# tum-pbs/PhiFlow

Measured on NVIDIA H100. Metric: smoke_plume_512^3_steps_per_sec, higher is better.
Workload: dtype f32

## Files before the change

phiflow_b200/csrc/ring_kernels.cu:

```cuda
#include <cooperative_groups.h>
#include <type_traits>
#include "cg_common.cuh"
#include <cstdlib>
#include <cstring>
#include "launch.cuh"

namespace cg = cooperative_groups;

#define RING_CONSUMERS 256
#define RING_THREADS (RING_CONSUMERS + 32)
#define RING_MAX_STAGES 8
#define RING_G 4

struct RingCfg {
    int TY, R, pitch, nx4;
    int stage_floats;
    int ZC, nyt, nzc;
    int units_per_batch, total_units;
    int consumers;
    int groups;
    int shfl_ok;
    int hint;
    int merge;
    int dbg;
    int split, Zm, split_t;
};

__device__ __forceinline__ uint32_t smem_u32(const void* p) { return (uint32_t)__cvta_generic_to_shared(p); }
__device__ __forceinline__ void mbar_init(uint32_t bar, uint32_t count)
{ asm volatile("mbarrier.init.shared::cta.b64 [%0], %1;" ::"r"(bar), "r"(count) : "memory"); }
__device__ __forceinline__ void mbar_expect_tx(uint32_t bar, uint32_t bytes)
{ asm volatile("mbarrier.arrive.expect_tx.shared::cta.b64 _, [%0], %1;" ::"r"(bar), "r"(bytes) : "memory"); }
__device__ __forceinline__ void mbar_arrive(uint32_t bar)
{ asm volatile("mbarrier.arrive.shared::cta.b64 _, [%0];" ::"r"(bar) : "memory"); }
__device__ __forceinline__ void mbar_wait(uint32_t bar, uint32_t parity)
{
    asm volatile(
        "{\n"
        ".reg .pred p;\n"
        "WAIT_LOOP:\n"
        "mbarrier.try_wait.parity.shared::cta.b64 p, [%0], %1;\n"
        "@p bra.uni WAIT_DONE;\n"
        "bra.uni WAIT_LOOP;\n"
        "WAIT_DONE:\n"
        "}\n" ::"r"(bar), "r"(parity) : "memory");
}
__device__ __forceinline__ void bulk_g2s(uint32_t dst, const void* src, uint32_t bytes, uint32_t bar)
{
    asm volatile("cp.async.bulk.shared::cluster.global.mbarrier::complete_tx::bytes [%0], [%1], %2, [%3];"
                 ::"r"(dst), "l"(src), "r"(bytes), "r"(bar) : "memory");
}
__device__ __forceinline__ void bulk_g2s_stream(uint32_t dst, const void* src, uint32_t bytes, uint32_t bar)
{
    uint64_t pol;
    asm volatile("createpolicy.fractional.L2::evict_first.b64 %0, 1.0;" : "=l"(pol));
    asm volatile("cp.async.bulk.shared::cluster.global.mbarrier::complete_tx::bytes.L2::cache_hint [%0], [%1], %2, [%3], %4;"
                 ::"r"(dst), "l"(src), "r"(bytes), "r"(bar), "l"(pol) : "memory");
}
__device__ __forceinline__ void fence_proxy_async() { asm volatile("fence.proxy.async;" ::: "memory"); }

struct SlotIt {
    int slot; unsigned par;
    __device__ __forceinline__ void next(int R) { if (++slot == R) { slot = 0; par ^= 1u; } }
};

struct Ring {
    float* stage0;
    uint32_t stage0_s, full0, empty0;
    SlotIt pos;
};

__device__ __forceinline__ void ring_init(Ring& rg, unsigned char* smem, const RingCfg& cfg)
{
    uint64_t* bars = reinterpret_cast<uint64_t*>(smem);
    rg.full0 = smem_u32(bars);
    rg.empty0 = smem_u32(bars + RING_MAX_STAGES);
    rg.stage0 = reinterpret_cast<float*>(smem + 128);
    rg.stage0_s = smem_u32(rg.stage0);
    rg.pos.slot = 0; rg.pos.par = 0;
    if (threadIdx.x == 0) {
        for (int s = 0; s < cfg.R; ++s) {
            mbar_init(rg.full0 + 8 * s, 1);
            mbar_init(rg.empty0 + 8 * s, cfg.consumers / 32);
        }
        asm volatile("fence.mbarrier_init.release.cluster;" ::: "memory");
    }
    __syncthreads();
}

struct ProdUnit {
    long long yoff[4];
    const float* base[4];
    uint32_t dsto[4];
    uint32_t nbytes[4];
    unsigned hmask, emask;
    int tot_h, tot_e;
};

template <int DIM, bool KSLOT = false>
__device__ __forceinline__ void prod_unit_setup(ProdUnit& pu, const RingCfg& cfg, const DGrid& g, const DField& pf,
                                                unsigned hactive, int NHslots, int NE, const float* const* hsrc, const float* const* esrc,
                                                int b, int y0, int kb = 0)
{
    const int lane = threadIdx.x & 31, hrows = cfg.TY + 2;
    const uint32_t row_bytes = (uint32_t)cfg.pitch * 4u;
    const bool mergeable = cfg.merge && pf.sy == cfg.pitch;
    pu.hmask = pu.emask = 0;
    int ch = 0, ce = 0;
#pragma unroll
    for (int it = 0; it < 4; ++it) {
        const int r = lane + 32 * it;
        pu.yoff[it] = 0; pu.base[it] = nullptr; pu.dsto[it] = 0; pu.nbytes[it] = row_bytes;
        int key = -1, yv = 0;
        bool halo_line = false;
        if (r < NHslots * hrows) {
            const int arr = r / hrows, j = r - arr * hrows;
            int yy = y0 - 1 + j; float cv;
            if (((hactive >> arr) & 1u) && yy <= g.n[1] && phi_resolve(yy, pf, 1, cv)) {
                pu.yoff[it] = (long long)((KSLOT && arr == NHslots - 1) ? kb : b) * pf.sb + (long long)yy * pf.sy;
                pu.base[it] = hsrc[arr];
                pu.dsto[it] = 4u * (uint32_t)((arr * hrows + j) * cfg.pitch);
                key = arr; yv = yy; halo_line = true; ch++;
            }
        } else if (r < NHslots * hrows + NE * cfg.TY) {
            const int q = r - NHslots * hrows, arr = q / cfg.TY, j = q - arr * cfg.TY;
            const int yy = y0 + j;
            if (yy < g.n[1]) {
                pu.yoff[it] = (long long)b * pf.sb + (long long)yy * pf.sy;
                pu.base[it] = esrc[arr];
                pu.dsto[it] = 4u * (uint32_t)((NHslots * hrows + arr * cfg.TY + j) * cfg.pitch);
                key = 8 + arr; yv = yy; ce++;
            }
        }
        const int pkey = __shfl_up_sync(0xffffffffu, key, 1), pyv = __shfl_up_sync(0xffffffffu, yv, 1);
        const bool cont = mergeable && key >= 0 && lane > 0 && pkey == key && pyv + 1 == yv;
        const unsigned cm = __ballot_sync(0xffffffffu, cont);
        if (key >= 0 && !cont) {
            const unsigned follow = lane == 31 ? 0u : (cm >> (lane + 1));
            pu.nbytes[it] = (uint32_t)__ffs(~follow) * row_bytes;
            if (halo_line) pu.hmask |= 1u << it; else pu.emask |= 1u << it;
        }
    }
#pragma unroll
    for (int o = 16; o > 0; o >>= 1) { ch += __shfl_xor_sync(0xffffffffu, ch, o); ce += __shfl_xor_sync(0xffffffffu, ce, o); }
    pu.tot_h = ch; pu.tot_e = ce;
}

template <int DIM>
__device__ __forceinline__ void ring_produce(Ring& rg, const RingCfg& cfg, const DField& pf, const ProdUnit& pu, int z, bool interior)
{
    const int lane = threadIdx.x & 31;
    const int slot = rg.pos.slot;
    const uint32_t full = rg.full0 + 8 * slot;
    const uint32_t row_bytes = (uint32_t)cfg.pitch * 4u;
    const uint32_t sbase = rg.stage0_s + 4u * (uint32_t)(slot * cfg.stage_floats);
    float cv;
    bool zmem = true;
    if (DIM == 3) zmem = phi_resolve(z, pf, 2, cv); else z = 0;
    const long long zoff = (long long)z * pf.sz;
    unsigned mask = (zmem ? pu.hmask : 0u) | (interior ? pu.emask : 0u);
    const int cnt = (zmem ? pu.tot_h : 0) + (interior ? pu.tot_e : 0);
    if (lane == 0) {
        mbar_wait(rg.empty0 + 8 * slot, rg.pos.par ^ 1u);
        if (cnt > 0) mbar_expect_tx(full, (uint32_t)cnt * row_bytes); else mbar_arrive(full);
    }
    __syncwarp();
#pragma unroll
    for (int it = 0; it < 4; ++it)
        if (mask & (1u << it)) {
            if (cfg.hint && (pu.emask & (1u << it))) bulk_g2s_stream(sbase + pu.dsto[it], pu.base[it] + pu.yoff[it] + zoff, pu.nbytes[it], full);
            else bulk_g2s(sbase + pu.dsto[it], pu.base[it] + pu.yoff[it] + zoff, pu.nbytes[it], full);
        }
    rg.pos.next(cfg.R);
}

__device__ __forceinline__ void ring_wait_full(const Ring& rg, const SlotIt& s) { mbar_wait(rg.full0 + 8 * s.slot, s.par); }
__device__ __forceinline__ void ring_release(const Ring& rg, const SlotIt& s)
{
    __syncwarp();
    if ((threadIdx.x & 31) == 0) mbar_arrive(rg.empty0 + 8 * s.slot);
}
__device__ __forceinline__ const float* ring_ptr(const Ring& rg, const RingCfg& cfg, const SlotIt& s)
{ return rg.stage0 + (size_t)s.slot * cfg.stage_floats; }

#define GF_VALID 1u
#define GF_XLO   2u
#define GF_XHI   4u
#define GF_YLOC  8u
#define GF_YHIC  16u

struct ThreadGroups {
    int soff[RING_G];
    int eoff[RING_G];
    int goff[RING_G];
    int j[RING_G];
    int xlo[RING_G], xro[RING_G];
    unsigned needl, needr;
    unsigned flags[RING_G];
    bool fast_ok;
};

__device__ __forceinline__ void groups_init(ThreadGroups& tg, const RingCfg& cfg, const DGrid& g, const DField& pf)
{
    const int lane = threadIdx.x & 31, nx = g.n[0];
    tg.needl = tg.needr = 0;
#pragma unroll
    for (int k = 0; k < RING_G; ++k) {
        const int gi = threadIdx.x + k * cfg.consumers;
        const int j = gi / cfg.nx4, x0 = (gi - j * cfg.nx4) * 4;
        tg.j[k] = (k < cfg.groups && j < cfg.TY && x0 < nx) ? j : -1;
        tg.soff[k] = (j + 1) * cfg.pitch + x0;
        tg.eoff[k] = j * cfg.pitch + x0;
        tg.goff[k] = j * (int)pf.sy + x0;
        tg.flags[k] = 0;
        const int row = (j + 1) * cfg.pitch;
        tg.xlo[k] = tg.soff[k] - 1; tg.xro[k] = tg.soff[k] + 4;
        if (lane == 0) tg.needl |= 1u << k;
        if (lane == 31) tg.needr |= 1u << k;
        if (x0 == 0) { tg.needl |= 1u << k; tg.xlo[k] = pf.klo[0] == PHI_BC_PERIODIC ? row + nx - 1 : row; }
        if (x0 + 4 >= nx) { tg.needr |= 1u << k; tg.xro[k] = pf.khi[0] == PHI_BC_PERIODIC ? row : row + nx - 1; }
        if (!(tg.needl & (1u << k))) tg.xlo[k] = 0;
        if (!(tg.needr & (1u << k))) tg.xro[k] = 0;
    }
    tg.fast_ok = cfg.shfl_ok && (cfg.nx4 * 4 == nx) && (cfg.TY * cfg.nx4 == cfg.groups * cfg.consumers)
                 && pf.klo[0] != PHI_BC_CONST && pf.khi[0] != PHI_BC_CONST;
}

__device__ __forceinline__ void groups_tile(ThreadGroups& tg, const RingCfg& cfg, const DGrid& g, const DField& pf, int y0)
{
    const int nx = g.n[0], ny = g.n[1];
#pragma unroll
    for (int k = 0; k < RING_G; ++k) {
        unsigned f = 0;
        if (tg.j[k] >= 0) {
            const int y = y0 + tg.j[k];
            const int x0 = tg.eoff[k] - tg.j[k] * cfg.pitch;
            if (y < ny) {
                f = GF_VALID;
                if (x0 == 0) f |= GF_XLO;
                if (x0 + 4 >= nx) f |= GF_XHI;
                if (y == 0 && pf.klo[1] == PHI_BC_CONST) f |= GF_YLOC;
                if (y == ny - 1 && pf.khi[1] == PHI_BC_CONST) f |= GF_YHIC;
            }
        }
        tg.flags[k] = f;
    }
}

template <int DIM, int NH, int NE, CgOp OP = CgOp::Poisson, class Epi>
__device__ __forceinline__ void ring_compute(const RingCfg& cfg, const DGrid& g, const DField& pf, const ThreadGroups& tg,
                                             const float* sm, const float* sc, const float* sp, float beta,
                                             long long plane_off, int z, Epi& epi, const CgOperator* od)
{
    const int pitch = cfg.pitch;
    const int h1 = (cfg.TY + 2) * pitch;
    const int aoff = NH * (cfg.TY + 2) * pitch;
    const int e0off = (NH + (cg_op_xslot(OP) ? 1 : 0)) * (cfg.TY + 2) * pitch;
    const int e1off = e0off + cfg.TY * pitch;
    const float ix2 = g.inv_dx2[0], iy2 = g.inv_dx2[1], iz2 = g.inv_dx2[2];
    const bool zm_const = DIM == 3 && z == 0 && pf.klo[2] == PHI_BC_CONST;
    const bool zp_const = DIM == 3 && z == g.n[2] - 1 && pf.khi[2] == PHI_BC_CONST;
    const bool use1 = NH == 2 && beta != 0.f;
    const int lane = threadIdx.x & 31;

    auto val4 = [&](const float* s, int off) -> float4 {
        float4 a = *reinterpret_cast<const float4*>(s + off);
        if (use1) { const float4 o = *reinterpret_cast<const float4*>(s + h1 + off);
                    a.x = fmaf(beta, o.x, a.x); a.y = fmaf(beta, o.y, a.y); a.z = fmaf(beta, o.z, a.z); a.w = fmaf(beta, o.w, a.w); }
        return a;
    };
    auto val1 = [&](const float* s, int off) -> float {
        float a = s[off];
        if (use1) a = fmaf(beta, s[h1 + off], a);
        return a;
    };

#pragma unroll
    for (int k = 0; k < RING_G; ++k) {
        const unsigned f = tg.flags[k];
        const int rc = tg.soff[k];
        const bool valid = (f & GF_VALID) != 0;
        float4 c = f4_splat(0.f);
        if (valid) c = val4(sc, rc);
        float xl, xr;
        if (cfg.shfl_ok) {
            xl = __shfl_up_sync(0xffffffffu, c.w, 1);
            xr = __shfl_down_sync(0xffffffffu, c.x, 1);
            if (valid && lane == 0 && !(f & GF_XLO)) xl = val1(sc, rc - 1);
            if (valid && lane == 31 && !(f & GF_XHI)) xr = val1(sc, rc + 4);
        } else if (valid) {
            xl = (f & GF_XLO) ? 0.f : val1(sc, rc - 1);
            xr = (f & GF_XHI) ? 0.f : val1(sc, rc + 4);
        }
        if (!valid) continue;
        float4 ym, yp, q;
        int nvalid = 4;
        if (f == GF_VALID) {
            ym = val4(sc, rc - pitch);
            yp = val4(sc, rc + pitch);
        } else {
            const int row = rc - (tg.eoff[k] - tg.j[k] * pitch);
            const int nx = g.n[0];
            const int x0 = rc - row;
            nvalid = min(4, nx - x0);
            ym = (f & GF_YLOC) ? f4_splat(pf.clo[1]) : val4(sc, rc - pitch);
            yp = (f & GF_YHIC) ? f4_splat(pf.chi[1]) : val4(sc, rc + pitch);
            if (f & GF_XLO) { const int kx = pf.klo[0]; xl = kx == PHI_BC_PERIODIC ? val1(sc, row + nx - 1) : (kx == PHI_BC_ZERO_GRADIENT ? c.x : pf.clo[0]); }
            if (f & GF_XHI) { const int kx = pf.khi[0]; xr = kx == PHI_BC_PERIODIC ? val1(sc, row) : (kx == PHI_BC_ZERO_GRADIENT ? f4_get(c, nvalid - 1) : pf.chi[0]); }
        }
        float4 r4 = make_float4(c.y, c.z, c.w, xr);
        if (nvalid < 4) f4_set(r4, nvalid - 1, xr);
        if constexpr (cg_op_xslot(OP)) {
            const float* am = sm + aoff; const float* ac_ = sc + aoff; const float* ap = sp + aoff;
            auto cw = [od](float v) { return OP == CgOp::Masked ? v : __fmul_rn(od->ndt, v); };
            auto cw4 = [&](const float* p) { const float4 v = *reinterpret_cast<const float4*>(p); return make_float4(cw(v.x), cw(v.y), cw(v.z), cw(v.w)); };
            auto glo = [od](int ax) { return OP == CgOp::Masked ? 1.f : od->kclo[ax]; };
            auto ghi = [od](int ax) { return OP == CgOp::Masked ? 1.f : od->kchi[ax]; };
            const float4 ac = cw4(ac_ + rc);
            const int row = rc - (tg.eoff[k] - tg.j[k] * pitch);
            const int nx = g.n[0];
            float axl = (f & GF_XLO) ? (pf.klo[0] == PHI_BC_PERIODIC ? cw(ac_[row + nx - 1]) : (pf.klo[0] == PHI_BC_ZERO_GRADIENT ? ac.x : glo(0))) : cw(ac_[rc - 1]);
            float axr = (f & GF_XHI) ? (pf.khi[0] == PHI_BC_PERIODIC ? cw(ac_[row]) : (pf.khi[0] == PHI_BC_ZERO_GRADIENT ? f4_get(ac, nvalid - 1) : ghi(0))) : cw(ac_[rc + 4]);
            const float4 al4 = make_float4(axl, ac.x, ac.y, ac.z);
            float4 ar4 = make_float4(ac.y, ac.z, ac.w, axr);
            if (nvalid < 4) f4_set(ar4, nvalid - 1, axr);
            const float4 l4 = make_float4(xl, c.x, c.y, c.z);
            const float4 aym = (f & GF_YLOC) ? f4_splat(glo(1)) : cw4(ac_ + rc - pitch);
            const float4 ayp = (f & GF_YHIC) ? f4_splat(ghi(1)) : cw4(ac_ + rc + pitch);
            auto term = [](float vn, float vc, float an, float a0) { return fminf(an, a0) * (vn - vc); };
            q.x = (term(l4.x, c.x, al4.x, ac.x) + term(r4.x, c.x, ar4.x, ac.x)) * ix2 + (term(ym.x, c.x, aym.x, ac.x) + term(yp.x, c.x, ayp.x, ac.x)) * iy2;
            q.y = (term(l4.y, c.y, al4.y, ac.y) + term(r4.y, c.y, ar4.y, ac.y)) * ix2 + (term(ym.y, c.y, aym.y, ac.y) + term(yp.y, c.y, ayp.y, ac.y)) * iy2;
            q.z = (term(l4.z, c.z, al4.z, ac.z) + term(r4.z, c.z, ar4.z, ac.z)) * ix2 + (term(ym.z, c.z, aym.z, ac.z) + term(yp.z, c.z, ayp.z, ac.z)) * iy2;
            q.w = (term(l4.w, c.w, al4.w, ac.w) + term(r4.w, c.w, ar4.w, ac.w)) * ix2 + (term(ym.w, c.w, aym.w, ac.w) + term(yp.w, c.w, ayp.w, ac.w)) * iy2;
            if (DIM == 3) {
                const float4 zm = zm_const ? f4_splat(pf.clo[2]) : val4(sm, rc);
                const float4 zp = zp_const ? f4_splat(pf.chi[2]) : val4(sp, rc);
                const float4 azm = zm_const ? f4_splat(glo(2)) : cw4(am + rc);
                const float4 azp = zp_const ? f4_splat(ghi(2)) : cw4(ap + rc);
                q.x += (term(zm.x, c.x, azm.x, ac.x) + term(zp.x, c.x, azp.x, ac.x)) * iz2;
                q.y += (term(zm.y, c.y, azm.y, ac.y) + term(zp.y, c.y, azp.y, ac.y)) * iz2;
                q.z += (term(zm.z, c.z, azm.z, ac.z) + term(zp.z, c.z, azp.z, ac.z)) * iz2;
                q.w += (term(zm.w, c.w, azm.w, ac.w) + term(zp.w, c.w, azp.w, ac.w)) * iz2;
            }
            if constexpr (OP == CgOp::Masked) {
                if (ac.x == 0.f) q.x = c.x;
                if (ac.y == 0.f) q.y = c.y;
                if (ac.z == 0.f) q.z = c.z;
                if (ac.w == 0.f) q.w = c.w;
                epi.set_acc(ac);
            }
        } else {
        q.x = (xl + r4.x - 2.f * c.x) * ix2 + (ym.x + yp.x - 2.f * c.x) * iy2;
        q.y = (c.x + r4.y - 2.f * c.y) * ix2 + (ym.y + yp.y - 2.f * c.y) * iy2;
        q.z = (c.y + r4.z - 2.f * c.z) * ix2 + (ym.z + yp.z - 2.f * c.z) * iy2;
        q.w = (c.z + r4.w - 2.f * c.w) * ix2 + (ym.w + yp.w - 2.f * c.w) * iy2;
        if (DIM == 3) {
            const float4 zm = zm_const ? f4_splat(pf.clo[2]) : val4(sm, rc);
            const float4 zp = zp_const ? f4_splat(pf.chi[2]) : val4(sp, rc);
            q.x += (zm.x + zp.x - 2.f * c.x) * iz2;
            q.y += (zm.y + zp.y - 2.f * c.y) * iz2;
            q.z += (zm.z + zp.z - 2.f * c.z) * iz2;
            q.w += (zm.w + zp.w - 2.f * c.w) * iz2;
        }
        }
        float4 e0 = f4_splat(0.f), e1 = f4_splat(0.f), e2 = f4_splat(0.f);
        if (NE >= 1) e0 = *reinterpret_cast<const float4*>(sc + e0off + tg.eoff[k]);
        if (NE >= 2) e1 = *reinterpret_cast<const float4*>(sc + e1off + tg.eoff[k]);
        if (NE >= 3) e2 = *reinterpret_cast<const float4*>(sc + e1off + cfg.TY * pitch + tg.eoff[k]);
        epi(plane_off + tg.goff[k], c, q, nvalid, e0, e1, e2);
    }
}

struct ZMarch { float4 m[2], c[2]; bool have; };

template <int DIM, int NH, int NE, int G, bool MARCH, class Epi>
__device__ __forceinline__ void ring_compute_fast(const RingCfg& cfg, const DGrid& g, const ThreadGroups& tg,
                                                  const float* sm, const float* sc, const float* sp, float beta,
                                                  long long plane_off, Epi& epi, ZMarch& zs)
{
    const int pitch = cfg.pitch;
    const int h1 = (cfg.TY + 2) * pitch;
    const int e0off = NH * (cfg.TY + 2) * pitch;
    const int e1off = e0off + cfg.TY * pitch;
    const float ix2 = g.inv_dx2[0], iy2 = g.inv_dx2[1], iz2 = DIM == 3 ? g.inv_dx2[2] : 0.f;
    const float cc = 2.f * (ix2 + iy2 + iz2);
    const bool use1 = NH == 2 && beta != 0.f;
    auto val4 = [&](const float* s, int off) -> float4 {
        float4 a = *reinterpret_cast<const float4*>(s + off);
        if (use1) { const float4 o = *reinterpret_cast<const float4*>(s + h1 + off);
                    a.x = fmaf(beta, o.x, a.x); a.y = fmaf(beta, o.y, a.y); a.z = fmaf(beta, o.z, a.z); a.w = fmaf(beta, o.w, a.w); }
        return a;
    };
#pragma unroll
    for (int k = 0; k < G; ++k) {
        const int rc = tg.soff[k];
        constexpr bool MZ = MARCH && DIM == 3 && G <= 2;
        const float4 c = (MZ && zs.have) ? zs.c[k & 1] : val4(sc, rc);
        const float4 ym = val4(sc, rc - pitch);
        const float4 yp = val4(sc, rc + pitch);
        float xl = __shfl_up_sync(0xffffffffu, c.w, 1);
        float xr = __shfl_down_sync(0xffffffffu, c.x, 1);
        if (MARCH) {
            float el = sc[tg.xlo[k]], er = sc[tg.xro[k]];
            if (use1) { el = fmaf(beta, sc[h1 + tg.xlo[k]], el); er = fmaf(beta, sc[h1 + tg.xro[k]], er); }
            xl = (tg.needl & (1u << k)) ? el : xl;
            xr = (tg.needr & (1u << k)) ? er : xr;
        } else {
            if (tg.needl & (1u << k)) { xl = sc[tg.xlo[k]]; if (use1) xl = fmaf(beta, sc[h1 + tg.xlo[k]], xl); }
            if (tg.needr & (1u << k)) { xr = sc[tg.xro[k]]; if (use1) xr = fmaf(beta, sc[h1 + tg.xro[k]], xr); }
        }
        float4 q;
        q.x = fmaf(ix2, xl + c.y, fmaf(iy2, ym.x + yp.x, -cc * c.x));
        q.y = fmaf(ix2, c.x + c.z, fmaf(iy2, ym.y + yp.y, -cc * c.y));
        q.z = fmaf(ix2, c.y + c.w, fmaf(iy2, ym.z + yp.z, -cc * c.z));
        q.w = fmaf(ix2, c.z + xr, fmaf(iy2, ym.w + yp.w, -cc * c.w));
        if (DIM == 3) {
            const float4 zm = (MZ && zs.have) ? zs.m[k & 1] : val4(sm, rc);
            const float4 zp = val4(sp, rc);
            q.x = fmaf(iz2, zm.x + zp.x, q.x);
            q.y = fmaf(iz2, zm.y + zp.y, q.y);
            q.z = fmaf(iz2, zm.z + zp.z, q.z);
            q.w = fmaf(iz2, zm.w + zp.w, q.w);
            if (MZ) { zs.m[k & 1] = c; zs.c[k & 1] = zp; }
        }
        float4 e0 = f4_splat(0.f), e1 = f4_splat(0.f), e2 = f4_splat(0.f);
        if (NE >= 1) e0 = *reinterpret_cast<const float4*>(sc + e0off + tg.eoff[k]);
        if (NE >= 2) e1 = *reinterpret_cast<const float4*>(sc + e1off + tg.eoff[k]);
        if (NE >= 3) e2 = *reinterpret_cast<const float4*>(sc + e1off + cfg.TY * pitch + tg.eoff[k]);
        epi(plane_off + tg.goff[k], c, q, 4, e0, e1, e2);
    }
    zs.have = MARCH && DIM == 3 && G <= 2;
}

template <bool GENERIC, int DIM, int NH, int NE, bool MARCH, CgOp OP, class Epi>
__device__ __forceinline__ void ring_compute_any(const RingCfg& cfg, const DGrid& g, const DField& pf, const ThreadGroups& tg,
                                                 bool fast, const float* sm, const float* sc, const float* sp, float beta,
                                                 long long plane_off, int z, Epi& epi, ZMarch& zs, const CgOperator* od)
{
    if (cfg.dbg & 4) return;
    if (cg_op_xslot(OP)) { zs.have = false; ring_compute<DIM, NH, NE, OP>(cfg, g, pf, tg, sm, sc, sp, beta, plane_off, z, epi, od); return; }
    if (!GENERIC || fast) {
        if (cfg.groups == 4) { ring_compute_fast<DIM, NH, NE, 4, MARCH>(cfg, g, tg, sm, sc, sp, beta, plane_off, epi, zs); return; }
        if (cfg.groups == 2) { ring_compute_fast<DIM, NH, NE, 2, MARCH>(cfg, g, tg, sm, sc, sp, beta, plane_off, epi, zs); return; }
        if (cfg.groups == 1) { ring_compute_fast<DIM, NH, NE, 1, MARCH>(cfg, g, tg, sm, sc, sp, beta, plane_off, epi, zs); return; }
    }
    zs.have = false;
    if (GENERIC) ring_compute<DIM, NH, NE>(cfg, g, pf, tg, sm, sc, sp, beta, plane_off, z, epi, od);
}

struct RingUnit { int b, y0, z0, z1; };

template <int DIM>
__device__ __forceinline__ RingUnit ring_unit(const RingCfg& cfg, const DGrid& g, int unit)
{
    RingUnit u;
    u.b = unit / cfg.units_per_batch;
    const int r = unit - u.b * cfg.units_per_batch;
    if (DIM == 3) { const int zc = r / cfg.nyt, yt = r - zc * cfg.nyt; u.y0 = yt * cfg.TY; u.z0 = zc * cfg.ZC; u.z1 = min(g.n[2], u.z0 + cfg.ZC); }
    else { u.y0 = r * cfg.TY; u.z0 = 0; u.z1 = 1; }
    return u;
}

template <int DIM>
__device__ __forceinline__ bool ring_next_unit(const RingCfg& cfg, const DGrid& g, int k, RingUnit& u)
{
    if (!cfg.split) {
        const int unit = blockIdx.x + k * gridDim.x;
        if (unit >= cfg.total_units) return false;
        u = ring_unit<DIM>(cfg, g, unit);
        return true;
    }
    if ((int)blockIdx.x < cfg.nyt) {
        if (k > 0) return false;
        u.b = 0; u.y0 = blockIdx.x * cfg.TY; u.z0 = 0; u.z1 = cfg.Zm;
        return true;
    }
    const int t = ((int)blockIdx.x - cfg.nyt) * cfg.split_t + k;
    if (k >= cfg.split_t || t >= cfg.nyt) return false;
    u.b = 0; u.y0 = t * cfg.TY; u.z0 = cfg.Zm; u.z1 = g.n[2];
    return true;
}

template <bool GENERIC, int NH, int NE, bool MARCH, int G, CgOp OP, class Epi>
__device__ __forceinline__ void ring_consume_planes(Ring& rg, const RingCfg& cfg, const DGrid& g, const DField& pf, const ThreadGroups& tg,
                                                    bool tile_fast, float beta, long long plane_off, const RingUnit& u, Epi& epi,
                                                    const CgOperator* od)
{
    const int nz = u.z1 - u.z0;
    SlotIt a = rg.pos, bq = a; bq.next(cfg.R);
    SlotIt c2 = bq; c2.next(cfg.R);
    ZMarch zs; zs.have = false;
    ring_wait_full(rg, a); ring_wait_full(rg, bq);
    for (int zi = 0; zi < nz; ++zi) {
        const int z = u.z0 + zi;
        ring_wait_full(rg, c2);
        epi.set_plane(z, g.n[2]);
        if (G > 0) {
            if (!(cfg.dbg & 4))
                ring_compute_fast<3, NH, NE, (G > 0 ? G : 1), MARCH>(cfg, g, tg, ring_ptr(rg, cfg, a), ring_ptr(rg, cfg, bq), ring_ptr(rg, cfg, c2),
                                                                     beta, plane_off, epi, zs);
        } else {
            const bool fast = tile_fast && !(z == 0 && pf.klo[2] == PHI_BC_CONST) && !(z == g.n[2] - 1 && pf.khi[2] == PHI_BC_CONST);
            ring_compute_any<GENERIC, 3, NH, NE, MARCH, OP>(cfg, g, pf, tg, fast, ring_ptr(rg, cfg, a), ring_ptr(rg, cfg, bq), ring_ptr(rg, cfg, c2),
                                                            beta, plane_off, z, epi, zs, od);
        }
        ring_release(rg, a);
        a = bq; bq = c2; c2.next(cfg.R);
        plane_off += pf.sz;
    }
    ring_release(rg, a); ring_release(rg, bq);
    rg.pos = c2;
}

template <bool GENERIC, int DIM, int NH, int NE, bool MARCH = true, CgOp OP = CgOp::Poisson, class Epi>
__device__ __forceinline__ void ring_process_unit(Ring& rg, const RingCfg& cfg, const DGrid& g, const DField& pf,
                                                  ThreadGroups& tg,
                                                  const float* const* hsrc, const float* const* esrc, float beta,
                                                  const RingUnit& u, Epi& epi, int kb = 0, const CgOperator* od = nullptr)
{
    constexpr bool XSLOT = cg_op_xslot(OP);
    const bool producer = (int)threadIdx.x >= cfg.consumers;
    if (producer) {
        const int nh = (NH == 2 && beta == 0.f) ? 1 : NH;
        ProdUnit pu;
        prod_unit_setup<DIM, OP == CgOp::HelmholtzVarying>(pu, cfg, g, pf, ((1u << nh) - 1u) | (XSLOT ? (1u << NH) : 0u), NH + (XSLOT ? 1 : 0), NE, hsrc, esrc, u.b, u.y0, kb);
        if (DIM == 3) {
            const int nz = u.z1 - u.z0;
            for (int p = 0; p < nz + 2; ++p)
                ring_produce<DIM>(rg, cfg, pf, pu, u.z0 - 1 + p, p >= 1 && p <= nz);
        } else {
            ring_produce<DIM>(rg, cfg, pf, pu, 0, true);
        }
        return;
    }
    const int ny = g.n[1];
    const bool tile_fast = !XSLOT && (!GENERIC || tg.fast_ok && u.y0 + cfg.TY <= ny
                           && !(u.y0 == 0 && pf.klo[1] == PHI_BC_CONST) && !(u.y0 + cfg.TY == ny && pf.khi[1] == PHI_BC_CONST));
    if (GENERIC) groups_tile(tg, cfg, g, pf, u.y0);
    long long plane_off = (long long)u.b * pf.sb + (long long)u.y0 * pf.sy + (DIM == 3 ? (long long)u.z0 * pf.sz : 0);
    if (DIM == 3) {
        if (!GENERIC && cfg.groups == 2) ring_consume_planes<GENERIC, NH, NE, MARCH, 2, OP>(rg, cfg, g, pf, tg, tile_fast, beta, plane_off, u, epi, od);
        else if (!GENERIC && cfg.groups == 4) ring_consume_planes<GENERIC, NH, NE, MARCH, 4, OP>(rg, cfg, g, pf, tg, tile_fast, beta, plane_off, u, epi, od);
        else if (!GENERIC) ring_consume_planes<GENERIC, NH, NE, MARCH, 1, OP>(rg, cfg, g, pf, tg, tile_fast, beta, plane_off, u, epi, od);
        else ring_consume_planes<GENERIC, NH, NE, MARCH, 0, OP>(rg, cfg, g, pf, tg, tile_fast, beta, plane_off, u, epi, od);
    } else {
        const SlotIt a = rg.pos;
        ring_wait_full(rg, a);
        const float* sc = ring_ptr(rg, cfg, a);
        epi.set_plane(-1, 0);
        ZMarch zs; zs.have = false;
        ring_compute_any<GENERIC, DIM, NH, NE, MARCH, OP>(cfg, g, pf, tg, tile_fast, sc, sc, sc, beta, plane_off, 0, epi, zs, od);
        ring_release(rg, a);
        rg.pos.next(cfg.R);
    }
}

struct NoPeerHalo {
    int zf;
    __device__ __forceinline__ void set_plane(int, int) {}
    __device__ __forceinline__ void put4(long long, const float4&) const {}
    __device__ __forceinline__ void put1(long long, float) const {}
};

struct PeerHalo {
    float* plo; float* phi; int zf;
    __device__ __forceinline__ void set_plane(int z, int nz) { zf = ((z == 0 && plo) ? 1 : 0) | ((z == nz - 1 && phi) ? 2 : 0); }
    __device__ __forceinline__ void put4(long long off, const float4& v) const
    {
        if (zf & 1) *reinterpret_cast<float4*>(plo + off) = v;
        if (zf & 2) *reinterpret_cast<float4*>(phi + off) = v;
    }
    __device__ __forceinline__ void put1(long long off, float v) const
    {
        if (zf & 1) plo[off] = v;
        if (zf & 2) phi[off] = v;
    }
};

template <bool AXPY>
struct REpiLaplace {
    float* y; float coeff;
    __device__ __forceinline__ void set_plane(int, int) {}
    __device__ __forceinline__ void set_acc(const float4&) {}
    __device__ __forceinline__ void operator()(long long off, const float4& c, const float4& q, int nvalid, const float4&, const float4&, const float4&)
    {
        float4 o = q;
        if (AXPY) { o.x = c.x + coeff * q.x; o.y = c.y + coeff * q.y; o.z = c.z + coeff * q.z; o.w = c.w + coeff * q.w; }
        if (nvalid == 4) *reinterpret_cast<float4*>(y + off) = o;
        else for (int j = 0; j < nvalid; ++j) y[off + j] = f4_get(o, j);
    }
};

template <class PH>
struct REpiResidual0 {
    float* r; float mean, offs; float acc0, acc1; PH ph; bool tol_from_y;
    float4 am = make_float4(1.f, 1.f, 1.f, 1.f);
    __device__ __forceinline__ void set_plane(int z, int nz) { ph.set_plane(z, nz); }
    __device__ __forceinline__ void set_acc(const float4& a) { am = a; }
    __device__ __forceinline__ void operator()(long long off, const float4& c, const float4& q, int nvalid, const float4& y, const float4&, const float4&)
    {
        float4 rt = make_float4((y.x - mean * am.x) - q.x, (y.y - mean * am.y) - q.y, (y.z - mean * am.z) - q.z, (y.w - mean * am.w) - q.w);
        float4 rr = make_float4(rt.x - offs, rt.y - offs, rt.z - offs, rt.w - offs);
        if (tol_from_y) rt = make_float4(y.x - mean * am.x, y.y - mean * am.y, y.z - mean * am.z, y.w - mean * am.w);
        if (nvalid == 4) {
            *reinterpret_cast<float4*>(r + off) = rr;
            if (ph.zf) ph.put4(off, rr);
            acc0 += rr.x * rr.x + rr.y * rr.y + rr.z * rr.z + rr.w * rr.w;
            acc1 += rt.x * rt.x + rt.y * rt.y + rt.z * rt.z + rt.w * rt.w;
        } else for (int j = 0; j < nvalid; ++j) { const float a = f4_get(rr, j), t = f4_get(rt, j); r[off + j] = a; if (ph.zf) ph.put1(off + j, a); acc0 += a * a; acc1 += t * t; }
    }
};

template <class PH>
struct REpiPassA {
    __device__ __forceinline__ void set_acc(const float4&) {}
    float* dnew; float acc0, acc1; PH ph;
    __device__ __forceinline__ void set_plane(int z, int nz) { ph.set_plane(z, nz); }
    __device__ __forceinline__ void operator()(long long off, const float4& c, const float4& q, int nvalid, const float4&, const float4&, const float4&)
    {
        if (nvalid == 4) {
            *reinterpret_cast<float4*>(dnew + off) = c;
            if (ph.zf) ph.put4(off, c);
            acc0 += c.x * q.x + c.y * q.y + c.z * q.z + c.w * q.w;
            acc1 += (c.x + c.y) + (c.z + c.w);
        } else for (int j = 0; j < nvalid; ++j) { const float v = f4_get(c, j); dnew[off + j] = v; if (ph.zf) ph.put1(off + j, v); acc0 += v * f4_get(q, j); acc1 += v; }
    }
};

template <class PH>
struct REpiPassAAdapt {
    __device__ __forceinline__ void set_acc(const float4&) {}
    float* dnew; float acc0, acc1; PH ph;
    __device__ __forceinline__ void set_plane(int z, int nz) { ph.set_plane(z, nz); }
    __device__ __forceinline__ void operator()(long long off, const float4& c, const float4& q, int nvalid, const float4& re, const float4&, const float4&)
    {
        if (nvalid == 4) {
            *reinterpret_cast<float4*>(dnew + off) = c;
            if (ph.zf) ph.put4(off, c);
            acc0 += c.x * q.x + c.y * q.y + c.z * q.z + c.w * q.w;
            acc1 += c.x * re.x + c.y * re.y + c.z * re.z + c.w * re.w;
        } else for (int j = 0; j < nvalid; ++j) { const float v = f4_get(c, j); dnew[off + j] = v; if (ph.zf) ph.put1(off + j, v); acc0 += v * f4_get(q, j); acc1 += v * f4_get(re, j); }
    }
};

template <class PH, bool RQ = false>
struct REpiPassBr {
    __device__ __forceinline__ void set_acc(const float4&) {}
    float* r; float alpha, offs; float acc0, acc1; PH ph;
    __device__ __forceinline__ void set_plane(int z, int nz) { ph.set_plane(z, nz); }
    __device__ __forceinline__ void operator()(long long off, const float4& c, const float4& q, int nvalid, const float4& re, const float4&, const float4&)
    {
        float4 rv = re;
        rv.x -= alpha * (q.x + offs); rv.y -= alpha * (q.y + offs); rv.z -= alpha * (q.z + offs); rv.w -= alpha * (q.w + offs);
        if (nvalid == 4) {
            *reinterpret_cast<float4*>(r + off) = rv;
            if (ph.zf) ph.put4(off, rv);
            acc0 += rv.x * rv.x + rv.y * rv.y + rv.z * rv.z + rv.w * rv.w;
            if (RQ) acc1 += rv.x * q.x + rv.y * q.y + rv.z * q.z + rv.w * q.w;
        } else for (int j = 0; j < nvalid; ++j) { const float t = f4_get(rv, j); r[off + j] = t; if (ph.zf) ph.put1(off + j, t); acc0 += t * t; if (RQ) acc1 += t * f4_get(q, j); }
    }
};

template <class PH, bool RQ = false>
struct REpiPassB {
    __device__ __forceinline__ void set_acc(const float4&) {}
    float* x; float* r; float alpha, aprev, offs; float acc0, acc1; PH ph;
    __device__ __forceinline__ void set_plane(int z, int nz) { ph.set_plane(z, nz); }
    __device__ __forceinline__ void operator()(long long off, const float4& c, const float4& q, int nvalid, const float4& xe, const float4& re, const float4& dp)
    {
        float4 xv = xe, rv = re;
        xv.x += aprev * dp.x; xv.y += aprev * dp.y; xv.z += aprev * dp.z; xv.w += aprev * dp.w;
        xv.x += alpha * c.x; xv.y += alpha * c.y; xv.z += alpha * c.z; xv.w += alpha * c.w;
        rv.x -= alpha * (q.x + offs); rv.y -= alpha * (q.y + offs); rv.z -= alpha * (q.z + offs); rv.w -= alpha * (q.w + offs);
        if (nvalid == 4) {
            *reinterpret_cast<float4*>(x + off) = xv;
            *reinterpret_cast<float4*>(r + off) = rv;
            if (ph.zf) ph.put4(off, rv);
            acc0 += rv.x * rv.x + rv.y * rv.y + rv.z * rv.z + rv.w * rv.w;
            if (RQ) acc1 += rv.x * q.x + rv.y * q.y + rv.z * q.z + rv.w * q.w;
        } else for (int j = 0; j < nvalid; ++j) { x[off + j] = f4_get(xv, j); const float t = f4_get(rv, j); r[off + j] = t; if (ph.zf) ph.put1(off + j, t); acc0 += t * t; if (RQ) acc1 += t * f4_get(q, j); }
    }
};

template <class Epi>
struct REpiHelm {
    Epi& e; float a;
    __device__ __forceinline__ void set_plane(int z, int nz) { e.set_plane(z, nz); }
    __device__ __forceinline__ void set_acc(const float4& m) { e.set_acc(m); }
    __device__ __forceinline__ void operator()(long long off, const float4& c, const float4& q, int nvalid, const float4& e0, const float4& e1, const float4& e2)
    {
        const float4 m = make_float4(fmaf(-a, q.x, c.x), fmaf(-a, q.y, c.y), fmaf(-a, q.z, c.z), fmaf(-a, q.w, c.w));
        e(off, c, m, nvalid, e0, e1, e2);
    }
};

template <class Epi>
struct REpiVarHelm {
    Epi& e;
    __device__ __forceinline__ void set_plane(int z, int nz) { e.set_plane(z, nz); }
    __device__ __forceinline__ void set_acc(const float4&) {}
    __device__ __forceinline__ void operator()(long long off, const float4& c, const float4& q, int nvalid, const float4& e0, const float4& e1, const float4& e2)
    {
        const float4 m = make_float4(c.x + q.x, c.y + q.y, c.z + q.z, c.w + q.w);
        e(off, c, m, nvalid, e0, e1, e2);
    }
};

template <int DIM, bool AXPY, bool GENERIC>
__global__ void __launch_bounds__(RING_THREADS, 2)
k_laplace_ring(DGrid g, DField f, RingCfg cfg, const float* __restrict__ x, float* __restrict__ y, float coeff)
{
    extern __shared__ __align__(128) unsigned char smem[];
    Ring rg;
    ring_init(rg, smem, cfg);
    ThreadGroups tg;
    groups_init(tg, cfg, g, f);
    const float* hsrc[2] = {x, nullptr};
    const float* esrc[2] = {nullptr, nullptr};
    REpiLaplace<AXPY> epi{y, coeff};
    for (int unit = blockIdx.x; unit < cfg.total_units; unit += gridDim.x) {
        const RingUnit u = ring_unit<DIM>(cfg, g, unit);
        ring_process_unit<GENERIC, DIM, 1, 0, false>(rg, cfg, g, f, tg, hsrc, esrc, 0.f, u, epi);
    }
}

struct CgRingArgs {
    CgArgs a;
    RingCfg cfg;
    int ring_smem_offset;
    int comm_merge;
    CommDev cm;
    float* d2;
    CgOperator op;
};

template <int DIM, bool GENERIC, CgOp OP, int NH, int NE, class Epi>
__device__ __forceinline__ void cg_op_unit(Ring& rg, const CgRingArgs& A, ThreadGroups& tg, const float* const* hsrc,
                                           const float* const* esrc, float beta, const RingUnit& u, Epi& epi)
{
    if constexpr (OP == CgOp::Helmholtz) {
        REpiHelm<Epi> he{epi, A.op.amount};
        ring_process_unit<GENERIC, DIM, NH, NE, true, OP>(rg, A.cfg, A.a.g, A.a.pf, tg, hsrc, esrc, beta, u, he);
    } else if constexpr (OP == CgOp::HelmholtzVarying) {
        REpiVarHelm<Epi> he{epi};
        ring_process_unit<GENERIC, DIM, NH, NE, true, OP>(rg, A.cfg, A.a.g, A.a.pf, tg, hsrc, esrc, beta, u, he, A.op.kbcast ? 0 : u.b, &A.op);
    } else ring_process_unit<GENERIC, DIM, NH, NE, true, OP>(rg, A.cfg, A.a.g, A.a.pf, tg, hsrc, esrc, beta, u, epi);
}

__device__ __forceinline__ unsigned long long ld_acquire_sys(const unsigned long long* p)
{
    unsigned long long v;
    asm volatile("ld.acquire.sys.global.u64 %0, [%1];" : "=l"(v) : "l"(p) : "memory");
    return v;
}
__device__ __forceinline__ void st_release_sys(unsigned long long* p, unsigned long long v)
{
    asm volatile("st.release.sys.global.u64 [%0], %1;" ::"l"(p), "l"(v) : "memory");
}

__device__ __forceinline__ bool comm_allreduce(const CommDev& cm, const CgShared& sh, int batch, unsigned long long seq)
{
    const int par = (int)(seq & 1ull);
    const size_t stride = 2 * (size_t)CG_MAX_BATCH;
    if (blockIdx.x == 0) {
        for (int q = 0; q < cm.n; ++q) {
            double* dst = cm.mbox[q] + ((size_t)par * PHI_MAX_RANKS + cm.rank) * stride;
            for (int b = threadIdx.x; b < batch; b += blockDim.x) { dst[b] = sh.sum0[b]; dst[CG_MAX_BATCH + b] = sh.sum1[b]; }
        }
        __threadfence_system();
        __syncthreads();
        if ((int)threadIdx.x < cm.n) st_release_sys(cm.flag[threadIdx.x] + par * PHI_MAX_RANKS + cm.rank, seq);
    }
    bool ok = true;
    if ((int)threadIdx.x < cm.n) {
        const unsigned long long* f = cm.flag[cm.rank] + par * PHI_MAX_RANKS + threadIdx.x;
        const long long t0 = clock64();
        while (ld_acquire_sys(f) < seq) {
            if (clock64() - t0 > 40000000000ll) { ok = false; break; }
        }
    }
    ok = __syncthreads_and(ok);
    const double* src = cm.mbox[cm.rank] + (size_t)par * PHI_MAX_RANKS * stride;
    for (int b = threadIdx.x; b < batch; b += blockDim.x) {
        double s0 = 0, s1 = 0;
        for (int q = 0; q < cm.n; ++q) {
            s0 += *(volatile const double*)(src + q * stride + b);
            s1 += *(volatile const double*)(src + q * stride + CG_MAX_BATCH + b);
        }
        sh.sum0[b] = s0; sh.sum1[b] = s1;
    }
    __syncthreads();
    return ok;
}

__device__ __forceinline__ bool comm_barrier_allreduce(const CommDev& cm, const CgShared& sh, const double* partials, int region, int batch,
                                                       int units_per_batch, const unsigned char* active, unsigned long long seq)
{
    const int par = (int)(seq & 1ull);
    const size_t stride = 2 * (size_t)CG_MAX_BATCH;
    __threadfence_system();
    __syncthreads();
    if (threadIdx.x == 0) {
        const unsigned prev = atomicAdd(cm.arrive, 1u);
        sh.any_cont[1] = ((prev + 1u) % gridDim.x == 0u) ? 1 : 0;
    }
    __syncthreads();
    if (sh.any_cont[1]) {
        __threadfence();
        reduce_partials(sh, partials, region, batch, units_per_batch, active);
        for (int q = 0; q < cm.n; ++q) {
            double* dst = cm.mbox[q] + ((size_t)par * PHI_MAX_RANKS + cm.rank) * stride;
            for (int b = threadIdx.x; b < batch; b += blockDim.x) { dst[b] = sh.sum0[b]; dst[CG_MAX_BATCH + b] = sh.sum1[b]; }
        }
        __threadfence_system();
        __syncthreads();
        if ((int)threadIdx.x < cm.n) st_release_sys(cm.flag[threadIdx.x] + par * PHI_MAX_RANKS + cm.rank, seq);
    }
    bool ok = true;
    if ((int)threadIdx.x < cm.n) {
        const unsigned long long* f = cm.flag[cm.rank] + par * PHI_MAX_RANKS + threadIdx.x;
        const long long t0 = clock64();
        while (ld_acquire_sys(f) < seq) {
            if (clock64() - t0 > 40000000000ll) { ok = false; break; }
        }
    }
    ok = __syncthreads_and(ok);
    const double* src = cm.mbox[cm.rank] + (size_t)par * PHI_MAX_RANKS * stride;
    for (int b = threadIdx.x; b < batch; b += blockDim.x) {
        double s0 = 0, s1 = 0;
        for (int q = 0; q < cm.n; ++q) {
            s0 += *(volatile const double*)(src + q * stride + b);
            s1 += *(volatile const double*)(src + q * stride + CG_MAX_BATCH + b);
        }
        sh.sum0[b] = s0; sh.sum1[b] = s1;
    }
    __syncthreads();
    return ok;
}

template <int DIM, class F>
__device__ __forceinline__ void ring_unit_cells(const RingCfg& cfg, const DGrid& g, const DField& pf, const ThreadGroups& tg,
                                                const RingUnit& u, F&& fn)
{
    if ((int)threadIdx.x >= cfg.consumers) return;
    long long plane_off = (long long)u.b * pf.sb + (long long)u.y0 * pf.sy + (DIM == 3 ? (long long)u.z0 * pf.sz : 0);
    for (int z = u.z0; z < u.z1; ++z, plane_off += pf.sz)
#pragma unroll
        for (int k = 0; k < RING_G; ++k) {
            if (tg.j[k] < 0 || u.y0 + tg.j[k] >= g.n[1]) continue;
            const int x0 = tg.eoff[k] - tg.j[k] * cfg.pitch;
            fn(plane_off + tg.goff[k], min(4, g.n[0] - x0));
        }
}

#define FUSED_GI 2
#define FUSED_GH 2
#define FUSED_TILE_BUFS 3

struct FusedGroups {
    int ti[FUSED_GI], th[FUSED_GH];
    int ei[FUSED_GI], eh[FUSED_GH];
    int gi[FUSED_GI];
    unsigned vi, vh;
};

__device__ __forceinline__ void fused_groups_init(FusedGroups& fg, const RingCfg& cfg, const DGrid& g, const DField& pf)
{
    const int lane = threadIdx.x & 31, nx = g.n[0], pitch = cfg.pitch, nx4 = cfg.nx4;
    auto edge = [&](int jj, int x0) -> int {
        const int row = jj * pitch;
        if (lane == 0) return x0 == 0 ? (pf.klo[0] == PHI_BC_PERIODIC ? row + nx - 1 : row) : row + x0 - 1;
        if (lane == 31) return x0 + 4 >= nx ? (pf.khi[0] == PHI_BC_PERIODIC ? row : row + nx - 1) : row + x0 + 4;
        return 0;
    };
    fg.vi = fg.vh = 0;
#pragma unroll
    for (int k = 0; k < FUSED_GI; ++k) {
        const int ge = threadIdx.x + k * cfg.consumers;
        const int j = ge / nx4, x0 = (ge - j * nx4) * 4;
        if (j < cfg.TY) fg.vi |= 1u << k;
        fg.ti[k] = (j + 1) * pitch + x0;
        fg.ei[k] = edge(j + 1, x0);
        fg.gi[k] = j * (int)pf.sy + x0;
    }
#pragma unroll
    for (int k = 0; k < FUSED_GH; ++k) {
        const int ge = threadIdx.x + k * cfg.consumers;
        const int h = ge / nx4, x0 = (ge - h * nx4) * 4;
        const int jj = h == 0 ? 0 : cfg.TY + 1;
        if (h < 2) fg.vh |= 1u << k;
        fg.th[k] = jj * pitch + x0;
        fg.eh[k] = edge(jj, x0);
    }
}

struct ProdUnitF {
    long long yoff[4];
    const float* base[4];
    uint32_t dsto[4];
    uint32_t nbytes[4];
    unsigned m[2];
    int tot[2];
};

__device__ __forceinline__ void prod_fused_setup(ProdUnitF& pu, const RingCfg& cfg, const DGrid& g, const DField& pf,
                                                 const float* d, const float* dprev, int b, int y0)
{
    const int lane = threadIdx.x & 31, TY = cfg.TY;
    const uint32_t row_bytes = (uint32_t)cfg.pitch * 4u;
    const bool mergeable = cfg.merge && pf.sy == cfg.pitch;
    const int rows[2] = {TY + 4, TY + 2};
    const int ylo[2] = {y0 - 2, y0 - 1};
    const float* src[2] = {d, dprev};
    int cnt[2] = {0, 0};
    pu.m[0] = pu.m[1] = 0;
#pragma unroll
    for (int it = 0; it < 4; ++it) {
        const int line = lane + 32 * it;
        pu.yoff[it] = 0; pu.base[it] = nullptr; pu.dsto[it] = 0; pu.nbytes[it] = row_bytes;
        int key = -1, yv = 0, first = 0;
#pragma unroll
        for (int arr = 0; arr < 2; ++arr) {
            if (key < 0 && line >= first && line < first + rows[arr] && src[arr]) {
                int yy = ylo[arr] + (line - first); float cv;
                phi_resolve(yy, pf, 1, cv);
                pu.yoff[it] = (long long)b * pf.sb + (long long)yy * pf.sy;
                pu.base[it] = src[arr];
                pu.dsto[it] = 4u * (uint32_t)(line * cfg.pitch);
                key = arr; yv = yy;
            }
            first += rows[arr];
        }
        cnt[0] += key == 0; cnt[1] += key == 1;
        const int pkey = __shfl_up_sync(0xffffffffu, key, 1), pyv = __shfl_up_sync(0xffffffffu, yv, 1);
        const bool cont = mergeable && key >= 0 && lane > 0 && pkey == key && pyv + 1 == yv;
        const unsigned cm = __ballot_sync(0xffffffffu, cont);
        if (key >= 0 && !cont) {
            const unsigned follow = lane == 31 ? 0u : (cm >> (lane + 1));
            pu.nbytes[it] = (uint32_t)__ffs(~follow) * row_bytes;
            pu.m[key] |= 1u << it;
        }
    }
#pragma unroll
    for (int c = 0; c < 2; ++c) {
#pragma unroll
        for (int o = 16; o > 0; o >>= 1) cnt[c] += __shfl_xor_sync(0xffffffffu, cnt[c], o);
        pu.tot[c] = cnt[c];
    }
}

__device__ __forceinline__ void ring_produce_fused(Ring& rg, const RingCfg& cfg, const DField& pf, const ProdUnitF& pu, int z, bool pplane)
{
    const int lane = threadIdx.x & 31;
    const int slot = rg.pos.slot;
    const uint32_t full = rg.full0 + 8 * slot;
    const uint32_t sbase = rg.stage0_s + 4u * (uint32_t)(slot * cfg.stage_floats);
    float cv;
    phi_resolve(z, pf, 2, cv);
    const long long zoff = (long long)z * pf.sz;
    const unsigned mask = pu.m[0] | (pplane ? pu.m[1] : 0u);
    const int cnt = pu.tot[0] + (pplane ? pu.tot[1] : 0);
    if (lane == 0) {
        mbar_wait(rg.empty0 + 8 * slot, rg.pos.par ^ 1u);
        mbar_expect_tx(full, (uint32_t)cnt * (uint32_t)cfg.pitch * 4u);
    }
    __syncwarp();
#pragma unroll
    for (int it = 0; it < 4; ++it)
        if (mask & (1u << it)) bulk_g2s(sbase + pu.dsto[it], pu.base[it] + pu.yoff[it] + zoff, pu.nbytes[it], full);
    rg.pos.next(cfg.R);
}

__device__ __forceinline__ float4 lds4(const float* s, int off) { return *reinterpret_cast<const float4*>(s + off); }
__device__ __forceinline__ float dot4(const float4& a, const float4& b) { return a.x * b.x + a.y * b.y + a.z * b.z + a.w * b.w; }

__device__ __forceinline__ float4 stencil7(const float4& c, float xl, float xr, const float4& ym, const float4& yp, const float4& zm, const float4& zp,
                                           float ix2, float iy2, float iz2, float cc)
{
    float4 q;
    q.x = fmaf(ix2, xl + c.y, fmaf(iy2, ym.x + yp.x, -cc * c.x));
    q.y = fmaf(ix2, c.x + c.z, fmaf(iy2, ym.y + yp.y, -cc * c.y));
    q.z = fmaf(ix2, c.y + c.w, fmaf(iy2, ym.z + yp.z, -cc * c.z));
    q.w = fmaf(ix2, c.z + xr, fmaf(iy2, ym.w + yp.w, -cc * c.w));
    q.x = fmaf(iz2, zm.x + zp.x, q.x);
    q.y = fmaf(iz2, zm.y + zp.y, q.y);
    q.z = fmaf(iz2, zm.z + zp.z, q.z);
    q.w = fmaf(iz2, zm.w + zp.w, q.w);
    return q;
}

struct FusedPass {
    const float* d; const float* dprev;
    float* dn; float* x;
    float alpha, aprev, beta, bprev;
};

__device__ __forceinline__ void ring_fused_unit(Ring& rg, const RingCfg& cfg, const DGrid& g, const DField& pf, const FusedGroups& fg,
                                                const FusedPass& P, float* tile, const RingUnit& u, float (&acc)[4])
{
    const int nz = u.z1 - u.z0;
    if ((int)threadIdx.x >= cfg.consumers) {
        ProdUnitF pu;
        prod_fused_setup(pu, cfg, g, pf, P.d, P.dprev, u.b, u.y0);
        for (int p = 0; p < nz + 4; ++p)
            ring_produce_fused(rg, cfg, pf, pu, u.z0 - 2 + p, p >= 1 && p <= nz + 2);
        return;
    }
    const int pitch = cfg.pitch, TY = cfg.TY;
    const int pb = (TY + 4) * pitch;
    const int tsz = (TY + 2) * pitch;
    const int lane = threadIdx.x & 31;
    const float ix2 = g.inv_dx2[0], iy2 = g.inv_dx2[1], iz2 = g.inv_dx2[2];
    const float cc = 2.f * (ix2 + iy2 + iz2);
    const float alpha = P.alpha, aprev = P.aprev, beta = P.beta, bprev = P.bprev;
    const bool has_prev = P.dprev != nullptr;
    long long plane_off = (long long)u.b * pf.sb + (long long)u.y0 * pf.sy + (long long)u.z0 * pf.sz - pf.sz;

    auto dnew = [&](const float* sc, const float* sn, int o, int e, const float4& c, const float4& zm, float4& rv, float4& dp, float4& zp) {
        const float4 ym = lds4(sc, o - pitch), yp = lds4(sc, o + pitch);
        zp = lds4(sn, o);
        float xl = __shfl_up_sync(0xffffffffu, c.w, 1), xr = __shfl_down_sync(0xffffffffu, c.x, 1);
        const float ev = sc[pitch + e];
        if (lane == 0) xl = ev;
        if (lane == 31) xr = ev;
        const float4 q = stencil7(c, xl, xr, ym, yp, zm, zp, ix2, iy2, iz2, cc);
        rv = c; dp = f4_splat(0.f);
        if (has_prev) {
            dp = lds4(sc, pb + o - pitch);
            rv = make_float4(fmaf(-bprev, dp.x, c.x), fmaf(-bprev, dp.y, c.y), fmaf(-bprev, dp.z, c.z), fmaf(-bprev, dp.w, c.w));
        }
        rv.x = fmaf(-alpha, q.x, rv.x); rv.y = fmaf(-alpha, q.y, rv.y); rv.z = fmaf(-alpha, q.z, rv.z); rv.w = fmaf(-alpha, q.w, rv.w);
        return make_float4(fmaf(beta, c.x, rv.x), fmaf(beta, c.y, rv.y), fmaf(beta, c.z, rv.z), fmaf(beta, c.w, rv.w));
    };

    float4 dm[FUSED_GI], dc[FUSED_GI];
    float4 hm[FUSED_GH], hc[FUSED_GH];
    float4 n2[FUSED_GI], n1[FUSED_GI];
    float4 r1[FUSED_GI];
    float4 xv[FUSED_GI];
    SlotIt cur = rg.pos, nxt = cur; nxt.next(cfg.R);
    ring_wait_full(rg, cur); ring_wait_full(rg, nxt);
    {
        const float* s0 = ring_ptr(rg, cfg, cur);
        const float* s1 = ring_ptr(rg, cfg, nxt);
#pragma unroll
        for (int k = 0; k < FUSED_GI; ++k) {
            dm[k] = dc[k] = n2[k] = n1[k] = r1[k] = xv[k] = f4_splat(0.f);
            if (fg.vi & (1u << k)) { dm[k] = lds4(s0, pitch + fg.ti[k]); dc[k] = lds4(s1, pitch + fg.ti[k]); }
        }
#pragma unroll
        for (int k = 0; k < FUSED_GH; ++k) {
            hm[k] = hc[k] = f4_splat(0.f);
            if (fg.vh & (1u << k)) { hm[k] = lds4(s0, pitch + fg.th[k]); hc[k] = lds4(s1, pitch + fg.th[k]); }
        }
    }
    ring_release(rg, cur);
    cur = nxt; nxt.next(cfg.R);
    for (int i = 0; i < nz + 2; ++i) {
        const bool own = i >= 1 && i <= nz;
        ring_wait_full(rg, nxt);
        const float* sc = ring_ptr(rg, cfg, cur);
        const float* sn = ring_ptr(rg, cfg, nxt);
        float* tw = tile + (i % FUSED_TILE_BUFS) * tsz;
#pragma unroll
        for (int k = 0; k < FUSED_GH; ++k) {
            if (!(fg.vh & (1u << k))) continue;
            float4 rv, dp, zp;
            const float4 dv = dnew(sc, sn, pitch + fg.th[k], fg.eh[k], hc[k], hm[k], rv, dp, zp);
            *reinterpret_cast<float4*>(tw + fg.th[k]) = dv;
            hm[k] = hc[k]; hc[k] = zp;
        }
        float4 n0[FUSED_GI], r0[FUSED_GI];
        float* const dnp = P.dn + plane_off;
        float* const xp = P.x ? P.x + plane_off : nullptr;
#pragma unroll
        for (int k = 0; k < FUSED_GI; ++k) {
            n0[k] = r0[k] = f4_splat(0.f);
            if (!(fg.vi & (1u << k))) continue;
            const float4 c = dc[k];
            float4 rv, dp, zp;
            const float4 dv = dnew(sc, sn, pitch + fg.ti[k], fg.ei[k], c, dm[k], rv, dp, zp);
            *reinterpret_cast<float4*>(tw + fg.ti[k]) = dv;
            if (own) {
                *reinterpret_cast<float4*>(dnp + fg.gi[k]) = dv;
                acc[1] += dot4(rv, rv);
                if (xp) {
                    float4 x4 = xv[k];
                    x4.x += aprev * dp.x; x4.y += aprev * dp.y; x4.z += aprev * dp.z; x4.w += aprev * dp.w;
                    x4.x += alpha * c.x; x4.y += alpha * c.y; x4.z += alpha * c.z; x4.w += alpha * c.w;
                    *reinterpret_cast<float4*>(xp + fg.gi[k]) = x4;
                }
            }
            n0[k] = dv; r0[k] = rv;
            dm[k] = c; dc[k] = zp;
        }
        ring_release(rg, cur);
        if (xp && i < nz) {
#pragma unroll
            for (int k = 0; k < FUSED_GI; ++k)
                if (fg.vi & (1u << k)) xv[k] = __ldcs(reinterpret_cast<const float4*>(xp + pf.sz + fg.gi[k]));
        }
        asm volatile("bar.sync 1, %0;" ::"r"(cfg.consumers) : "memory");
        if (i >= 2) {
            const float* tp = tile + ((i - 1) % FUSED_TILE_BUFS) * tsz;
#pragma unroll
            for (int k = 0; k < FUSED_GI; ++k) {
                if (!(fg.vi & (1u << k))) continue;
                const float4 c = n1[k];
                const float4 ym = lds4(tp, fg.ti[k] - pitch), yp = lds4(tp, fg.ti[k] + pitch);
                float xl = __shfl_up_sync(0xffffffffu, c.w, 1), xr = __shfl_down_sync(0xffffffffu, c.x, 1);
                const float ev = tp[fg.ei[k]];
                if (lane == 0) xl = ev;
                if (lane == 31) xr = ev;
                const float4 q = stencil7(c, xl, xr, ym, yp, n2[k], n0[k], ix2, iy2, iz2, cc);
                acc[0] += dot4(c, q);
                acc[2] += dot4(r1[k], q);
                acc[3] += dot4(q, q);
            }
        }
#pragma unroll
        for (int k = 0; k < FUSED_GI; ++k) { n2[k] = n1[k]; n1[k] = n0[k]; r1[k] = r0[k]; }
        cur = nxt; nxt.next(cfg.R);
        plane_off += pf.sz;
    }
    ring_release(rg, cur);
    rg.pos = nxt;
    asm volatile("bar.sync 1, %0;" ::"r"(cfg.consumers) : "memory");
}

struct REpiFusedStart {
    float* d; float acc0, acc1;
    __device__ __forceinline__ void set_plane(int, int) {}
    __device__ __forceinline__ void set_acc(const float4&) {}
    __device__ __forceinline__ void operator()(long long off, const float4& c, const float4& q, int, const float4&, const float4&, const float4&)
    {
        *reinterpret_cast<float4*>(d + off) = c;
        acc0 += dot4(c, q);
        acc1 += dot4(q, q);
    }
};

template <int DIM, bool GENERIC, bool DIST, bool ADAPT, CgOp OP = CgOp::Poisson, bool FUSED = false>
__global__ void __launch_bounds__(RING_THREADS, 1)
k_cg_ring(CgRingArgs A)
{
    constexpr bool MASK = OP == CgOp::Masked;
    static_assert((OP != CgOp::Helmholtz && OP != CgOp::HelmholtzVarying) || (!DIST && !ADAPT && !FUSED),
                  "the Helmholtz operators run on the single-GPU two-sweep CG only");
    static_assert(!MASK || !ADAPT || (!DIST && !FUSED), "CG-adaptive with obstacles runs on the single-GPU two-sweep CG only");
    static_assert(!cg_op_xslot(OP) || GENERIC, "the face-minimum stencil runs on the generic consumer");
    extern __shared__ __align__(128) unsigned char smem_raw[];
    const CgArgs& a = A.a;
    const RingCfg& cfg = A.cfg;
    CgShared sh = cg_carve(smem_raw, a.g.batch);
    Ring rg;
    ring_init(rg, smem_raw + A.ring_smem_offset, cfg);
    cg::grid_group grid = cg::this_grid();
    const DGrid& g = a.g;
    const int batch = g.batch;
    const double cells = (double)g.n[0] * g.n[1] * g.n[2] * (A.cm.n > 1 ? A.cm.n : 1);
    const float coffs = a.prm.matrix_offset;
    constexpr bool adaptive = ADAPT;
    int region = 0;
    ThreadGroups tg;
    groups_init(tg, cfg, g, a.pf);

    auto sweep = [&](const unsigned char* active, auto&& body) {
        int cur_b = cfg.split ? 0 : -1; float acc0 = 0.f, acc1 = 0.f;
        RingUnit u;
        for (int k = 0; ring_next_unit<DIM>(cfg, g, k, u); ++k) {
            if (active && !active[u.b]) continue;
            if (u.b != cur_b) {
                if (cur_b >= 0) flush_partials(sh, a.partials, region, batch, cur_b, acc0, acc1);
                cur_b = u.b; acc0 = 0.f; acc1 = 0.f;
            }
            body(u, acc0, acc1);
        }
        if (cur_b >= 0) flush_partials(sh, a.partials, region, batch, cur_b, acc0, acc1);
    };
    const CommDev& cm = A.cm;
    unsigned long long seq = cm.n > 1 ? *cm.seq : 0ull;
    bool comm_ok = true;
    auto barrier_and_reduce = [&](const unsigned char* active) {
        fence_proxy_async();
        if (DIST && cm.n > 1 && A.comm_merge) {
            comm_ok = comm_barrier_allreduce(cm, sh, a.partials, region, batch, cfg.split ? (int)gridDim.x : cfg.units_per_batch, active, ++seq) && comm_ok;
            region ^= 1;
            fence_proxy_async();
            return;
        }
        if (cm.n > 1) __threadfence_system();
        grid.sync();
        fence_proxy_async();
        reduce_partials(sh, a.partials, region, batch, cfg.split ? (int)gridDim.x : cfg.units_per_batch, active);
        region ^= 1;
        if (cm.n > 1) {
            comm_ok = comm_allreduce(cm, sh, batch, ++seq) && comm_ok;
            fence_proxy_async();
        }
    };
    const long long nzsz = (long long)g.n[2] * a.pf.sz;
    using PH = typename std::conditional<DIST, PeerHalo, NoPeerHalo>::type;
    auto peer_halo = [&](float* lo_arr, float* hi_arr) {
        PH ph;
        if constexpr (DIST) {
            ph.plo = cm.lower >= 0 ? lo_arr + nzsz : nullptr;
            ph.phi = cm.upper >= 0 ? hi_arr - nzsz : nullptr;
        }
        ph.zf = 0;
        return ph;
    };

    for (int b = threadIdx.x; b < batch; b += blockDim.x) { sh.mean[b] = 0.f; sh.offs[b] = 0.f; }
    __syncthreads();

    if (a.prm.balance_rhs || coffs != 0.f) {
        sweep(nullptr, [&](const RingUnit& u, float& acc0, float& acc1) {
            ring_unit_cells<DIM>(cfg, g, a.pf, tg, u, [&](long long off, int nvalid) {
                for (int j = 0; j < nvalid; ++j) { acc0 += a.rhs[off + j]; acc1 += MASK ? a.acc[off + j] : a.x[off + j]; }
            });
        });
        barrier_and_reduce(nullptr);
        for (int b = threadIdx.x; b < batch; b += blockDim.x) {
            if (MASK) { sh.mean[b] = (a.prm.balance_rhs && sh.sum1[b] > 0.0) ? (float)(sh.sum0[b] / sh.sum1[b]) : 0.f; sh.offs[b] = 0.f; }
            else { sh.mean[b] = a.prm.balance_rhs ? (float)(sh.sum0[b] / cells) : 0.f; sh.offs[b] = coffs * (float)sh.sum1[b]; }
        }
        __syncthreads();
    }

    {
        const float* hsrc[2] = {a.x, (OP == CgOp::Masked ? a.acc : (OP == CgOp::HelmholtzVarying ? A.op.k : nullptr))};
        const float* esrc[2] = {a.rhs, nullptr};
        sweep(nullptr, [&](const RingUnit& u, float& acc0, float& acc1) {
            REpiResidual0<PH> epi{a.r, sh.mean[u.b], sh.offs[u.b], 0.f, 0.f, peer_halo(cm.lo_r, cm.hi_r), adaptive};
            if constexpr (OP == CgOp::Poisson) ring_process_unit<GENERIC, DIM, 1, 1>(rg, cfg, g, a.pf, tg, hsrc, esrc, 0.f, u, epi);
            else cg_op_unit<DIM, GENERIC, OP, 1, 1>(rg, A, tg, hsrc, esrc, 0.f, u, epi);
            acc0 += epi.acc0; acc1 += epi.acc1;
        });
    }
    barrier_and_reduce(nullptr);
    for (int b = threadIdx.x; b < batch; b += blockDim.x) {
        const double d0 = sh.sum0[b], d0tol = sh.sum1[b];
        sh.delta[b] = d0;
        const float tol = fmaxf(a.prm.rtol * a.prm.rtol * (float)d0tol, a.prm.atol * a.prm.atol);
        sh.tol_sq[b] = tol; sh.rsq0[b] = (float)d0;
        const bool conv = (float)d0 <= tol;
        const bool divg = !isfinite((float)d0);
        sh.conv[b] = conv; sh.divg[b] = divg; sh.iters[b] = 0;
        sh.cont[b] = (!conv && !divg && a.prm.max_iter > 0) ? 1 : 0;
        sh.beta[b] = 0.f; sh.alpha[b] = 0.f; sh.aprev[b] = 0.f;
    }
    __syncthreads();
    if (threadIdx.x == 0) { int any = 0; for (int b = 0; b < batch; ++b) any |= sh.cont[b]; *sh.any_cont = any; }
    __syncthreads();

    if constexpr (FUSED) {
        static_assert(DIM == 3 && !GENERIC && !DIST && !ADAPT && OP == CgOp::Poisson, "the one-sweep CG is 3-D, branch-free, single-GPU CG only");
        float* const D[3] = {a.d0, a.d1, A.d2};
        float* const tile = rg.stage0 + (size_t)cfg.R * cfg.stage_floats;
        FusedGroups fg;
        fused_groups_init(fg, cfg, g, a.pf);
        if (*sh.any_cont) {
            const float* hsrc[2] = {a.r, nullptr};
            const float* esrc[2] = {nullptr, nullptr};
            sweep(sh.cont, [&](const RingUnit& u, float& acc0, float& acc1) {
                REpiFusedStart epi{D[0], 0.f, 0.f};
                ring_process_unit<false, 3, 1, 0, true>(rg, cfg, g, a.pf, tg, hsrc, esrc, 0.f, u, epi);
                acc0 += epi.acc0; acc1 += epi.acc1;
            });
            barrier_and_reduce(sh.cont);
            for (int b = threadIdx.x; b < batch; b += blockDim.x) {
                if (!sh.cont[b]) continue;
                const double dl = sh.delta[b], dq = sh.sum0[b];
                const float al = (dq != 0.0) ? (float)(dl / dq) : 0.f;
                const double nxt = dl - 2.0 * al * dq + (double)al * al * sh.sum1[b];
                sh.alpha[b] = al;
                sh.beta[b] = (dl != 0.0) ? (float)(nxt / dl) : 0.f;
                sh.bprev[b] = 0.f;
            }
            __syncthreads();
        }
        const int upb = cfg.split ? (int)gridDim.x : cfg.units_per_batch;
        int reg = 1;
        for (int k = 0; *sh.any_cont; ++k) {
            FusedPass P;
            P.d = D[k % 3]; P.dprev = k > 0 ? D[(k + 2) % 3] : nullptr;
            P.dn = D[(k + 1) % 3]; P.x = (k & 1) ? a.x : nullptr;
            int cur_b = cfg.split ? 0 : -1;
            float acc[4] = {0.f, 0.f, 0.f, 0.f};
            RingUnit u;
            for (int j = 0; ring_next_unit<3>(cfg, g, j, u); ++j) {
                if (!sh.cont[u.b]) continue;
                if (u.b != cur_b) {
                    if (cur_b >= 0) { flush_partials(sh, a.partials, 2 * reg, batch, cur_b, acc[0], acc[1]);
                                      flush_partials(sh, a.partials, 2 * reg + 1, batch, cur_b, acc[2], acc[3]); }
                    cur_b = u.b; acc[0] = acc[1] = acc[2] = acc[3] = 0.f;
                }
                P.alpha = sh.alpha[u.b]; P.aprev = sh.aprev[u.b]; P.beta = sh.beta[u.b]; P.bprev = sh.bprev[u.b];
                ring_fused_unit(rg, cfg, g, a.pf, fg, P, tile, u, acc);
            }
            if (cur_b >= 0) { flush_partials(sh, a.partials, 2 * reg, batch, cur_b, acc[0], acc[1]);
                              flush_partials(sh, a.partials, 2 * reg + 1, batch, cur_b, acc[2], acc[3]); }
            fence_proxy_async();
            grid.sync();
            fence_proxy_async();
            reduce_partials(sh, a.partials, 2 * reg, batch, upb, sh.cont);
            for (int b = threadIdx.x; b < batch; b += blockDim.x) {
                if (!sh.cont[b]) continue;
                const double dn = sh.sum1[b], dq = sh.sum0[b];
                sh.delta[b] = dn;
                const int it = ++sh.iters[b];
                const float rsq = fabsf((float)dn);
                const bool conv = rsq <= sh.tol_sq[b];
                const bool divg = !isfinite(rsq) || (rsq / sh.rsq0[b] > 1e5f && it >= 8);
                sh.conv[b] = conv; sh.divg[b] = divg;
                sh.cont[b] = (!conv && !divg && it < a.prm.max_iter) ? 1 : 0;
                if (sh.cont[b]) {
                    sh.aprev[b] = sh.alpha[b];
                    sh.bprev[b] = sh.beta[b];
                    sh.alpha[b] = (dq != 0.0) ? (float)(dn / dq) : 0.f;
                }
            }
            __syncthreads();
            reduce_partials(sh, a.partials, 2 * reg + 1, batch, upb, sh.cont);
            for (int b = threadIdx.x; b < batch; b += blockDim.x) {
                if (!sh.cont[b]) continue;
                const double dn = sh.delta[b], al = sh.alpha[b];
                const double nxt = dn - 2.0 * al * sh.sum0[b] + al * al * sh.sum1[b];
                sh.beta[b] = (dn != 0.0) ? (float)(nxt / dn) : 0.f;
            }
            __syncthreads();
            if (threadIdx.x == 0) { int any = 0; for (int b = 0; b < batch; ++b) any |= sh.cont[b]; *sh.any_cont = any; }
            __syncthreads();
            reg ^= 1;
        }
        region = reg == 1 ? 2 : 0;
        RingUnit u;
        for (int k = 0; ring_next_unit<DIM>(cfg, g, k, u); ++k) {
            const int it = sh.iters[u.b];
            if (!(it & 1)) continue;
            const float al = sh.alpha[u.b];
            const float* dl = D[(it - 1) % 3];
            ring_unit_cells<DIM>(cfg, g, a.pf, tg, u, [&](long long off, int) {
                float4 xv = *reinterpret_cast<const float4*>(a.x + off);
                const float4 dv = *reinterpret_cast<const float4*>(dl + off);
                xv.x += al * dv.x; xv.y += al * dv.y; xv.z += al * dv.z; xv.w += al * dv.w;
                *reinterpret_cast<float4*>(a.x + off) = xv;
            });
        }
    }

    float* dold = a.d0; float* dnew = a.d1;
    float* lo_dnew = cm.lo_d1; float* hi_dnew = cm.hi_d1; float* lo_dold = cm.lo_d0; float* hi_dold = cm.hi_d0;
    bool x_pending = false;
    while (!FUSED && *sh.any_cont && comm_ok) {
        if (cfg.dbg & 1) {} else if constexpr (!ADAPT) {
            const float* hsrc[3] = {a.r, dold, (OP == CgOp::Masked ? a.acc : (OP == CgOp::HelmholtzVarying ? A.op.k : nullptr))};
            const float* esrc[2] = {nullptr, nullptr};
            sweep(sh.cont, [&](const RingUnit& u, float& acc0, float& acc1) {
                REpiPassA<PH> epi{dnew, 0.f, 0.f, peer_halo(lo_dnew, hi_dnew)};
                if constexpr (OP == CgOp::Poisson) ring_process_unit<GENERIC, DIM, 2, 0>(rg, cfg, g, a.pf, tg, hsrc, esrc, sh.beta[u.b], u, epi);
                else cg_op_unit<DIM, GENERIC, OP, 2, 0>(rg, A, tg, hsrc, esrc, sh.beta[u.b], u, epi);
                acc0 += epi.acc0; acc1 += epi.acc1;
            });
        } else if constexpr (OP == CgOp::Poisson) {
            const float* hsrc[2] = {a.r, dold};
            const float* esrc[2] = {a.r, nullptr};
            sweep(sh.cont, [&](const RingUnit& u, float& acc0, float& acc1) {
                REpiPassAAdapt<PH> epi{dnew, 0.f, 0.f, peer_halo(lo_dnew, hi_dnew)};
                ring_process_unit<GENERIC, DIM, 2, 1>(rg, cfg, g, a.pf, tg, hsrc, esrc, sh.beta[u.b], u, epi);
                acc0 += epi.acc0; acc1 += epi.acc1;
            });
        } else {
            const float* hsrc[3] = {a.r, dold, a.acc};
            const float* esrc[2] = {a.r, nullptr};
            sweep(sh.cont, [&](const RingUnit& u, float& acc0, float& acc1) {
                REpiPassAAdapt<PH> epi{dnew, 0.f, 0.f, peer_halo(lo_dnew, hi_dnew)};
                cg_op_unit<DIM, GENERIC, OP, 2, 1>(rg, A, tg, hsrc, esrc, sh.beta[u.b], u, epi);
                acc0 += epi.acc0; acc1 += epi.acc1;
            });
        }
        barrier_and_reduce(sh.cont);
        for (int b = threadIdx.x; b < batch; b += blockDim.x) {
            if (!sh.cont[b]) continue;
            sh.aprev[b] = sh.alpha[b];
            if (adaptive) {
                const double dq = sh.sum0[b];
                sh.alpha[b] = (dq != 0.0) ? (float)(sh.sum1[b] / dq) : 0.f;
                sh.delta[b] = dq;
                sh.offs[b] = 0.f;
                continue;
            }
            const double S = sh.sum1[b];
            const double dq = sh.sum0[b] + (double)coffs * S * S;
            sh.alpha[b] = (dq != 0.0) ? (float)(sh.delta[b] / dq) : 0.f;
            sh.offs[b] = coffs * (float)S;
        }
        __syncthreads();
        if (cfg.dbg & 2) {} else if (!x_pending) {
            const float* hsrc[2] = {dnew, (OP == CgOp::Masked ? a.acc : (OP == CgOp::HelmholtzVarying ? A.op.k : nullptr))};
            const float* esrc[3] = {a.r, nullptr, nullptr};
            sweep(sh.cont, [&](const RingUnit& u, float& acc0, float& acc1) {
                REpiPassBr<PH, ADAPT> epi{a.r, sh.alpha[u.b], ADAPT ? 0.f : sh.offs[u.b], 0.f, 0.f, peer_halo(cm.lo_r, cm.hi_r)};
                if constexpr (OP == CgOp::Poisson) ring_process_unit<GENERIC, DIM, 1, 1>(rg, cfg, g, a.pf, tg, hsrc, esrc, 0.f, u, epi);
                else cg_op_unit<DIM, GENERIC, OP, 1, 1>(rg, A, tg, hsrc, esrc, 0.f, u, epi);
                acc0 += epi.acc0; if (ADAPT) acc1 += epi.acc1;
            });
        } else {
            const float* hsrc[2] = {dnew, (OP == CgOp::Masked ? a.acc : (OP == CgOp::HelmholtzVarying ? A.op.k : nullptr))};
            const float* esrc[3] = {a.x, a.r, dold};
            sweep(sh.cont, [&](const RingUnit& u, float& acc0, float& acc1) {
                REpiPassB<PH, ADAPT> epi{a.x, a.r, sh.alpha[u.b], sh.aprev[u.b], ADAPT ? 0.f : sh.offs[u.b], 0.f, 0.f, peer_halo(cm.lo_r, cm.hi_r)};
                if constexpr (OP == CgOp::Poisson) ring_process_unit<GENERIC, DIM, 1, 3>(rg, cfg, g, a.pf, tg, hsrc, esrc, 0.f, u, epi);
                else cg_op_unit<DIM, GENERIC, OP, 1, 3>(rg, A, tg, hsrc, esrc, 0.f, u, epi);
                acc0 += epi.acc0; if (ADAPT) acc1 += epi.acc1;
            });
        }
        x_pending = !x_pending;
        barrier_and_reduce(sh.cont);
        for (int b = threadIdx.x; b < batch; b += blockDim.x) {
            if (!sh.cont[b]) continue;
            const double dn = sh.sum0[b];
            const double dprev = sh.delta[b];
            if (adaptive) sh.beta[b] = (dprev != 0.0) ? -(float)(sh.sum1[b] / dprev) : 0.f;
            else sh.beta[b] = (dprev != 0.0) ? (float)(dn / dprev) : 0.f;
            sh.delta[b] = dn;
            const int it = ++sh.iters[b];
            const float rsq = fabsf((float)dn);
            const bool conv = rsq <= sh.tol_sq[b];
            const bool divg = !isfinite(rsq) || (rsq / sh.rsq0[b] > 1e5f && it >= 8);
            sh.conv[b] = conv; sh.divg[b] = divg;
            sh.cont[b] = (!conv && !divg && it < a.prm.max_iter) ? 1 : 0;
        }
        __syncthreads();
        if (threadIdx.x == 0) { int any = 0; for (int b = 0; b < batch; ++b) any |= sh.cont[b]; *sh.any_cont = any; }
        __syncthreads();
        float* t = dold; dold = dnew; dnew = t;
        t = lo_dold; lo_dold = lo_dnew; lo_dnew = t;
        t = hi_dold; hi_dold = hi_dnew; hi_dnew = t;
    }

    RingUnit u;
    for (int k = 0; !FUSED && ring_next_unit<DIM>(cfg, g, k, u); ++k) {
        if (!(sh.iters[u.b] & 1)) continue;
        const float al = sh.alpha[u.b];
        ring_unit_cells<DIM>(cfg, g, a.pf, tg, u, [&](long long off, int nvalid) {
            if (nvalid == 4) {
                float4 xv = *reinterpret_cast<const float4*>(a.x + off);
                const float4 dv = *reinterpret_cast<const float4*>(a.d1 + off);
                xv.x += al * dv.x; xv.y += al * dv.y; xv.z += al * dv.z; xv.w += al * dv.w;
                *reinterpret_cast<float4*>(a.x + off) = xv;
            } else for (int j = 0; j < nvalid; ++j) a.x[off + j] += al * a.d1[off + j];
        });
    }

    if (a.prm.project_mean) {
        sweep(nullptr, [&](const RingUnit& u, float& acc0, float& acc1) {
            ring_unit_cells<DIM>(cfg, g, a.pf, tg, u, [&](long long off, int nvalid) {
                for (int j = 0; j < nvalid; ++j) { if (MASK) { acc0 += a.x[off + j] * a.acc[off + j]; acc1 += a.acc[off + j]; } else acc0 += a.x[off + j]; }
            });
        });
        barrier_and_reduce(nullptr);
        for (int k = 0; ring_next_unit<DIM>(cfg, g, k, u); ++k) {
            const float m = MASK ? (sh.sum1[u.b] > 0.0 ? (float)(sh.sum0[u.b] / sh.sum1[u.b]) : 0.f) : (float)(sh.sum0[u.b] / cells);
            ring_unit_cells<DIM>(cfg, g, a.pf, tg, u, [&](long long off, int nvalid) {
                for (int j = 0; j < nvalid; ++j) a.x[off + j] -= MASK ? m * a.acc[off + j] : m;
            });
        }
    }

    if (cm.n > 1 && blockIdx.x == 0 && threadIdx.x == 0) *cm.seq = seq;
    if (blockIdx.x == 0) {
        for (int b = threadIdx.x; b < batch; b += blockDim.x) {
            PhiCgResult res;
            res.iterations = sh.iters[b]; res.converged = sh.conv[b]; res.diverged = comm_ok ? sh.divg[b] : -1;
            res.residual_sq = fabsf((float)sh.delta[b]); res.tol_sq = sh.tol_sq[b]; res.initial_residual_sq = sh.rsq0[b];
            a.result[b] = res;
        }
    }
}

static const int kSmemBudget = 227 * 1024;
#define RING_UNIT_OVERHEAD 2.5

static bool ring_config(const DGrid& g, int lines_a, int lines_b, int reserve_bytes, int min_stages, int max_stages,
                        int target_units, RingCfg* out, int consumers = RING_CONSUMERS, int zhalo = 2)
{
    RingCfg c;
    c.split = 0; c.Zm = 0; c.split_t = 0;
    c.consumers = consumers;
    c.pitch = g.cext[0]; c.nx4 = g.cext[0] / 4;
    const int row_bytes = c.pitch * 4;
    int ty = g.dim == 3 ? 4 : 16;
    if (g.dim == 3) {
        const int want = 2048 / (g.cext[0] > 0 ? g.cext[0] : 1);
        ty = 1;
        while (ty * 2 <= want && ty < 16) ty *= 2;
        while (ty > 1 && ty / 2 >= g.n[1]) ty /= 2;
    }
    if (const char* e = getenv("PHICUDA_RING_TY")) { const int v = atoi(e); if (v >= 1 && v <= 32) ty = v; }
    for (;; ty /= 2) {
        if (ty < 1) return false;
        if (ty * c.nx4 > RING_G * consumers) continue;
        if (lines_a * ty + lines_b > 128) continue;
        const int stage_bytes = (lines_a * ty + lines_b) * row_bytes;
        const int r = (kSmemBudget - reserve_bytes - 128) / stage_bytes;
        if (const char* e = getenv("PHICUDA_RING_R")) { const int v = atoi(e); if (v >= min_stages && v < max_stages) max_stages = v; }
        if (r >= min_stages) { c.TY = ty; c.R = r > max_stages ? max_stages : r; c.stage_floats = stage_bytes / 4; break; }
    }
    while (g.dim == 2 && c.TY > 1 && c.TY / 2 >= g.n[1]) c.TY /= 2;
    c.groups = (c.TY * c.nx4 + consumers - 1) / consumers;
    c.shfl_ok = (c.nx4 % 32 == 0) ? 1 : 0;
    { const char* e = getenv("PHICUDA_RING_HINT"); c.hint = (e && e[0] == '1') ? 1 : 0; }
    { const char* e = getenv("PHICUDA_RING_MERGE"); c.merge = (e && e[0] == '0') ? 0 : 1; }
    { const char* e = getenv("PHICUDA_RING_DEBUG"); c.dbg = e ? atoi(e) : 0; }
    if (g.dim == 3) {
        c.nyt = (g.n[1] + c.TY - 1) / c.TY;
        const int ctas = target_units;
        double best = -1.0; int best_nzc = 1;
        const int max_nzc = g.n[2] >= 4 ? g.n[2] / 4 : 1;
        for (int nzc = 1; nzc <= max_nzc; ++nzc) {
            const int zc = (g.n[2] + nzc - 1) / nzc;
            if ((g.n[2] + zc - 1) / zc != nzc) continue;
            const long long units = (long long)c.nyt * nzc * g.batch;
            const long long rounds = (units + ctas - 1) / ctas;
            const double util = (double)units / (double)(rounds * ctas);
            const double score = util / (1.0 + (zhalo + RING_UNIT_OVERHEAD) / zc);
            if (score > best + 1e-9) { best = score; best_nzc = nzc; }
        }
        if (const char* e = getenv("PHICUDA_RING_NZC")) {
            const int v = atoi(e);
            if (v >= 1 && v <= g.n[2]) { const int zc = (g.n[2] + v - 1) / v; best_nzc = (g.n[2] + zc - 1) / zc; }
        }
        c.nzc = best_nzc; c.ZC = (g.n[2] + best_nzc - 1) / best_nzc;
        c.units_per_batch = c.nyt * c.nzc;
        c.total_units = c.units_per_batch * g.batch;
    } else {
        c.nyt = (g.n[1] + c.TY - 1) / c.TY; c.nzc = 1; c.ZC = 1;
        c.units_per_batch = c.nyt; c.total_units = c.nyt * g.batch;
    }
    *out = c;
    return true;
}

static bool ring_all_fast(const DGrid& g, const DField& f, const RingCfg& c)
{
    if (!c.shfl_ok || c.nx4 * 4 != g.n[0] || c.TY * c.nx4 != c.groups * c.consumers || g.n[1] % c.TY != 0) return false;
    for (int a = 0; a < g.dim; ++a) if (f.klo[a] == PHI_BC_CONST || f.khi[a] == PHI_BC_CONST) return false;
    return c.groups == 1 || c.groups == 2 || c.groups == 4;
}

static void note_ring_launch(int kernel, const RingCfg& c, bool generic, bool dist, bool adaptive, int grid, bool masked = false)
{
    PhiLaunchInfo li; memset(&li, 0, sizeof(li));
    li.kernel = kernel; li.generic = generic; li.dist = dist; li.adaptive = adaptive; li.masked = masked;
    li.TY = c.TY; li.stages = c.R; li.ZC = c.ZC; li.nzc = c.nzc; li.groups = c.groups; li.total_units = c.total_units; li.grid_ctas = grid; li.split = c.split;
    phi_note_launch(li);
}

int phi_launch_laplace_ring(const DGrid& g, const DField& f, const float* x, float* y, float coeff, bool axpy, cudaStream_t s)
{
    RingCfg cfg;
    const int sms = phi_sm_count();
    if (!ring_config(g, 1, 2, kSmemBudget / 2 + 1024, g.dim == 3 ? 4 : 2, 6, sms * 2, &cfg)) return -100;
    const size_t smem = 128 + (size_t)cfg.R * cfg.stage_floats * 4;
    int grid = sms * 2;
    if (grid > cfg.total_units) grid = cfg.total_units;
    cudaError_t e;
    const bool generic = !ring_all_fast(g, f, cfg);
#define LAUNCH_LAP(D, AX, GEN) do { \
        e = cudaFuncSetAttribute(k_laplace_ring<D, AX, GEN>, cudaFuncAttributeMaxDynamicSharedMemorySize, (int)smem); \
        if (e == cudaSuccess) k_laplace_ring<D, AX, GEN><<<grid, RING_THREADS, smem, s>>>(g, f, cfg, x, y, coeff); } while (0)
#define LAUNCH_LAP2(D, AX) do { if (generic) LAUNCH_LAP(D, AX, true); else LAUNCH_LAP(D, AX, false); } while (0)
    if (g.dim == 3) { if (axpy) LAUNCH_LAP2(3, true); else LAUNCH_LAP2(3, false); }
    else            { if (axpy) LAUNCH_LAP2(2, true); else LAUNCH_LAP2(2, false); }
#undef LAUNCH_LAP2
#undef LAUNCH_LAP
    if (e != cudaSuccess) return (int)e;
    note_ring_launch(PHI_KERNEL_LAPLACE_RING, cfg, generic, false, false, grid);
    return (int)cudaGetLastError();
}

static bool cg_ring_config(const DGrid& g, CgOp op, int cgs, int target_units, RingCfg* c)
{
    const bool xslot = cg_op_xslot(op);
    return ring_config(g, xslot ? 5 : 4, xslot ? 6 : 2, cgs, g.dim == 3 ? (xslot ? 3 : 4) : 2, RING_MAX_STAGES, target_units, c);
}

using CgRingKernel = void (*)(CgRingArgs);
static CgRingKernel cg_ring_kernel(CgOp op, int dim, bool generic, bool dist, bool adapt, bool fused)
{
    constexpr CgOp P = CgOp::Poisson, M = CgOp::Masked, H = CgOp::Helmholtz, V = CgOp::HelmholtzVarying;
    const bool d3 = dim == 3;
    switch (op) {
    case P:
        if (fused)
            return d3 && !generic && !dist && !adapt ? k_cg_ring<3, false, false, false, P, true> : nullptr;
        if (d3) return generic ? (dist ? (adapt ? k_cg_ring<3, true, true, true> : k_cg_ring<3, true, true, false>)
                                       : (adapt ? k_cg_ring<3, true, false, true> : k_cg_ring<3, true, false, false>))
                               : (dist ? (adapt ? k_cg_ring<3, false, true, true> : k_cg_ring<3, false, true, false>)
                                       : (adapt ? k_cg_ring<3, false, false, true> : k_cg_ring<3, false, false, false>));
        return generic ? (dist ? (adapt ? k_cg_ring<2, true, true, true> : k_cg_ring<2, true, true, false>)
                               : (adapt ? k_cg_ring<2, true, false, true> : k_cg_ring<2, true, false, false>))
                       : (dist ? (adapt ? k_cg_ring<2, false, true, true> : k_cg_ring<2, false, true, false>)
                               : (adapt ? k_cg_ring<2, false, false, true> : k_cg_ring<2, false, false, false>));
    case M:
        if (!generic || fused || (adapt && dist)) return nullptr;
        if (adapt) return d3 ? k_cg_ring<3, true, false, true, M> : k_cg_ring<2, true, false, true, M>;
        return d3 ? (dist ? k_cg_ring<3, true, true, false, M> : k_cg_ring<3, true, false, false, M>)
                  : (dist ? k_cg_ring<2, true, true, false, M> : k_cg_ring<2, true, false, false, M>);
    case H:
        if (dist || adapt || fused) return nullptr;
        return d3 ? (generic ? k_cg_ring<3, true, false, false, H> : k_cg_ring<3, false, false, false, H>)
                  : (generic ? k_cg_ring<2, true, false, false, H> : k_cg_ring<2, false, false, false, H>);
    case V:
        if (dist || adapt || fused || !generic) return nullptr;
        return d3 ? k_cg_ring<3, true, false, false, V> : k_cg_ring<2, true, false, false, V>;
    }
    return nullptr;
}

int phi_launch_cg_ring(const CgLaunch& l, const CommDev* cm, cudaStream_t s)
{
    const DGrid& g = l.g;
    const CgOp op = l.op.kind;
    if (g.batch > CG_MAX_BATCH) return -100;
    if (op == CgOp::Masked && l.prm.matrix_offset != 0.f) return -100;
    const bool xslot = cg_op_xslot(op);
    CgRingArgs A;
    const int cgs = (int)((cg_smem_bytes(g.batch) + 127) / 128 * 128);
    const int sms = phi_sm_count();
    if (!cg_ring_config(g, op, cgs, sms, &A.cfg)) return -100;
    if (l.prm.method == PHI_SOLVER_CG_ADAPTIVE && !xslot && A.cfg.TY == 1
        && !ring_config(g, 4, 3, cgs, g.dim == 3 ? 4 : 2, RING_MAX_STAGES, sms, &A.cfg)) return -100;
    A.ring_smem_offset = cgs;
    int per_sm = 0;
    cudaError_t e;
    const bool generic = xslot || !ring_all_fast(g, l.pf, A.cfg);
    const bool dist = cm && cm->n > 1;
    const bool adapt = l.prm.method == PHI_SOLVER_CG_ADAPTIVE;
    bool fused = false;
    size_t tile_bytes = 0;
    {
        const char* e = getenv("PHICUDA_CG_PASSES");
        const DField& pf = l.pf;
        if (!(e && atoi(e) == 2) && g.dim == 3 && !generic && !dist && !adapt && op == CgOp::Poisson && l.prm.matrix_offset == 0.f
            && pf.klo[1] == PHI_BC_PERIODIC && pf.khi[1] == PHI_BC_PERIODIC && pf.klo[2] == PHI_BC_PERIODIC && pf.khi[2] == PHI_BC_PERIODIC) {
            RingCfg fc;
            if (ring_config(g, 3, 6, cgs, 4, RING_MAX_STAGES, sms, &fc, RING_CONSUMERS, 4)
                && ring_config(g, 3, 6, cgs + FUSED_TILE_BUFS * (fc.TY + 2) * fc.pitch * 4, 4, RING_MAX_STAGES, sms, &fc, RING_CONSUMERS, 4)
                && ring_all_fast(g, pf, fc) && fc.TY * fc.nx4 <= FUSED_GI * fc.consumers && 2 * fc.nx4 <= FUSED_GH * fc.consumers) {
                fused = true;
                A.cfg = fc;
                tile_bytes = (size_t)FUSED_TILE_BUFS * (fc.TY + 2) * fc.pitch * 4;
            }
        }
    }
    const int threads = RING_THREADS;
    const size_t smem = (size_t)cgs + 128 + (size_t)A.cfg.R * A.cfg.stage_floats * 4 + tile_bytes;
    const void* fn = (const void*)cg_ring_kernel(op, g.dim, generic, dist, adapt, fused);
    if (!fn) return -100;
    e = cudaFuncSetAttribute(fn, cudaFuncAttributeMaxDynamicSharedMemorySize, (int)smem);
    if (e == cudaSuccess) e = cudaOccupancyMaxActiveBlocksPerMultiprocessor(&per_sm, fn, threads, smem);
    if (e != cudaSuccess || per_sm < 1) return -100;
    int grid = sms * per_sm;
    A.cfg.split = 0; A.cfg.Zm = 0; A.cfg.split_t = 0;
    {
        const char* e = getenv("PHICUDA_RING_SPLIT");
        const int force = e ? atoi(e) : -1;
        const int nyt = A.cfg.nyt, nz = g.n[2];
        const int zh = fused ? 4 : 2;
        if (g.dim == 3 && g.batch == 1 && force != 0 && grid <= CG_MAX_GRID && nyt < grid && nz >= 8) {
            const int spare = grid - nyt, T = (nyt + spare - 1) / spare;
            int best_zm = 0; double best = 1e30;
            for (int zm = 4; zm <= nz - 1; ++zm) {
                const double main_c = zm + zh + RING_UNIT_OVERHEAD, tail_c = T * (nz - zm + zh + RING_UNIT_OVERHEAD);
                const double cost = main_c > tail_c ? main_c : tail_c;
                if (cost < best) { best = cost; best_zm = zm; }
            }
            const long long rounds = ((long long)A.cfg.total_units + grid - 1) / grid;
            const double dflt = rounds * (A.cfg.ZC + zh + RING_UNIT_OVERHEAD);
            if (best_zm > 0 && (force == 1 || best < dflt * 0.97)) {
                A.cfg.split = 1; A.cfg.Zm = best_zm; A.cfg.split_t = T;
                A.cfg.nzc = 2; A.cfg.ZC = best_zm; A.cfg.units_per_batch = A.cfg.total_units = 2 * nyt;
            }
        }
    }
    if (!A.cfg.split && grid > A.cfg.total_units) grid = A.cfg.total_units;
    if (grid > CG_MAX_GRID) grid = CG_MAX_GRID;
    const CgWorkspace w = phi_cg_workspace(g, l.workspace);
    CgArgs& a = A.a;
    a.g = g; a.pf = l.pf; a.um = UnitMap();
    a.rhs = l.rhs; a.x = l.x; a.acc = l.op.mask;
    a.r = w.r; a.d0 = w.d0; a.d1 = w.d1; a.partials = w.partials;
    A.d2 = w.d2;
    A.op = l.op;
    a.result = l.result; a.prm = l.prm;
    if (cm) A.cm = *cm; else { memset(&A.cm, 0, sizeof(A.cm)); A.cm.n = 1; A.cm.lower = A.cm.upper = -1; }
    { const char* e = getenv("PHICUDA_COMM_MERGE"); A.comm_merge = (e && e[0] == '1') ? 1 : 0; }
    void* args[] = {&A};
    e = cudaLaunchCooperativeKernel(fn, dim3(grid), dim3(threads), args, smem, s);
    if (e != cudaSuccess) { phi_set_error("cg ring: cooperative launch failed: %s", cudaGetErrorString(e)); return (int)e; }
    note_ring_launch(PHI_KERNEL_CG_RING, A.cfg, generic, dist, adapt, grid, op == CgOp::Masked);
    phi_note_cg_passes(fused ? 1 : 2);
    phi_note_cg_operator(op == CgOp::HelmholtzVarying ? PHI_CG_OP_HELMHOLTZ_VARYING : (op == CgOp::Helmholtz ? PHI_CG_OP_HELMHOLTZ : PHI_CG_OP_POISSON));
    return 0;
}

struct HelmConsts { float clo[3][3], chi[3][3]; };

__global__ void k_helm_bias(DGrid g, DField f, int C, float amount, HelmConsts hc, const float* __restrict__ y, float* __restrict__ out)
{
    const long long plane = (long long)g.n[0] * g.n[1], cells = plane * g.n[2], total = cells * g.batch;
    for (long long i = blockIdx.x * (long long)blockDim.x + threadIdx.x; i < total; i += (long long)gridDim.x * blockDim.x) {
        const int b = (int)(i / cells);
        const long long r = i - b * cells;
        const int z = (int)(r / plane), yy = (int)((r - z * plane) / g.n[0]), x = (int)(r - z * plane - (long long)yy * g.n[0]);
        const int idx[3] = {x, yy, z};
        const int c = b % C;
        float lap = 0.f;
        for (int ax = 0; ax < g.dim; ++ax) {
            float gs = 0.f;
            if (idx[ax] == 0 && f.klo[ax] == PHI_BC_CONST) gs += hc.clo[c][ax];
            if (idx[ax] == g.n[ax] - 1 && f.khi[ax] == PHI_BC_CONST) gs += hc.chi[c][ax];
            lap += gs * g.inv_dx2[ax];
        }
        const long long off = b * f.sb + z * f.sz + (long long)yy * f.sy + x;
        out[off] = fmaf(amount, lap, y[off]);
    }
}

__global__ void k_helm_bias_var(DGrid g, DField f, float ndt, HelmConsts hc, const float* __restrict__ k, int kbcast,
                                const float* __restrict__ y, float* __restrict__ out)
{
    const long long plane = (long long)g.n[0] * g.n[1], cells = plane * g.n[2], total = cells * g.batch;
    for (long long i = blockIdx.x * (long long)blockDim.x + threadIdx.x; i < total; i += (long long)gridDim.x * blockDim.x) {
        const int b = (int)(i / cells);
        const long long r = i - b * cells;
        const int z = (int)(r / plane), yy = (int)((r - z * plane) / g.n[0]), x = (int)(r - z * plane - (long long)yy * g.n[0]);
        const int idx[3] = {x, yy, z};
        const long long cell = z * f.sz + (long long)yy * f.sy + x;
        const float w = __fmul_rn(ndt, k[(kbcast ? 0 : b) * f.sb + cell]);
        float bias = 0.f;
        for (int ax = 0; ax < g.dim; ++ax) {
            float s = 0.f;
            if (idx[ax] == 0 && f.klo[ax] == PHI_BC_CONST) { const float c = hc.clo[0][ax]; s += fminf(w, c) * c; }
            if (idx[ax] == g.n[ax] - 1 && f.khi[ax] == PHI_BC_CONST) { const float c = hc.chi[0][ax]; s += fminf(w, c) * c; }
            bias += s * g.inv_dx2[ax];
        }
        const long long off = b * f.sb + cell;
        out[off] = y[off] - bias;
    }
}

bool phi_cg_ring_fits(const DGrid& g, CgOp op)
{
    if (g.batch > CG_MAX_BATCH || g.halo != 0) return false;
    RingCfg c;
    return cg_ring_config(g, op, (int)((cg_smem_bytes(g.batch) + 127) / 128 * 128), 1, &c);
}

int phi_cg_ring_max_width(const DGrid& g, CgOp op, bool adapt)
{
    if (g.batch > CG_MAX_BATCH || g.halo != 0) return 0;
    const int cgs = (int)((cg_smem_bytes(g.batch) + 127) / 128 * 128);
    for (int w = g.cext[0] < 4096 ? g.cext[0] / 4 * 4 : 4096; w >= 4; w -= 4) {
        DGrid h = g; h.n[0] = w; h.cext[0] = w;
        RingCfg c;
        if (!cg_ring_config(h, op, cgs, 1, &c)) continue;
        if (adapt && !cg_op_xslot(op) && c.TY == 1 && !ring_config(h, 4, 3, cgs, h.dim == 3 ? 4 : 2, RING_MAX_STAGES, 1, &c)) continue;
        return w;
    }
    return 0;
}

int phi_launch_diffuse_implicit(const CgLaunch& l, int C, const DField* cf, cudaStream_t s)
{
    const DGrid& g = l.g;
    const bool varying = l.op.kind == CgOp::HelmholtzVarying;
    HelmConsts hc;
    bool bias = false;
    for (int c = 0; c < 3; ++c)
        for (int ax = 0; ax < 3; ++ax) {
            const bool used = c < C && ax < g.dim;
            hc.clo[c][ax] = used && cf[c].klo[ax] == PHI_BC_CONST ? cf[c].clo[ax] : 0.f;
            hc.chi[c][ax] = used && cf[c].khi[ax] == PHI_BC_CONST ? cf[c].chi[ax] : 0.f;
            bias = bias || hc.clo[c][ax] != 0.f || hc.chi[c][ax] != 0.f;
        }
    CgLaunch m = l;
    if (bias && (varying || l.op.amount != 0.f)) {
        float* yb = phi_cg_workspace(g, l.workspace).d2;
        const long long total = (long long)g.n[0] * g.n[1] * g.n[2] * g.batch;
        const long long want = (total + 255) / 256, cap = (long long)phi_sm_count() * 8;
        const int blocks = (int)(want < cap ? want : cap);
        if (varying) k_helm_bias_var<<<blocks, 256, 0, s>>>(g, l.pf, l.op.ndt, hc, l.op.k, l.op.kbcast, l.rhs, yb);
        else k_helm_bias<<<blocks, 256, 0, s>>>(g, l.pf, C, l.op.amount, hc, l.rhs, yb);
        const cudaError_t e = cudaGetLastError();
        if (e != cudaSuccess) return (int)e;
        m.rhs = yb;
    }
    return phi_launch_cg_ring(m, nullptr, s);
}
```

Measured before the change: 1.979.

## Split fused CG ring kernel into register-rebalanced producer and consumer roles

```diff
diff --git a/phiflow_b200/csrc/cg_ring_body.cuh b/phiflow_b200/csrc/cg_ring_body.cuh
--- /dev/null
+++ b/phiflow_b200/csrc/cg_ring_body.cuh
@@ -0,0 +1,334 @@
+    constexpr bool MASK = OP == CgOp::Masked;
+    static_assert((OP != CgOp::Helmholtz && OP != CgOp::HelmholtzVarying) || (!DIST && !ADAPT && !FUSED),
+                  "the Helmholtz operators run on the single-GPU two-sweep CG only");
+    static_assert(!MASK || !ADAPT || (!DIST && !FUSED), "CG-adaptive with obstacles runs on the single-GPU two-sweep CG only");
+    static_assert(!cg_op_xslot(OP) || GENERIC, "the face-minimum stencil runs on the generic consumer");
+    extern __shared__ __align__(128) unsigned char smem_raw[];
+    const CgArgs& a = A.a;
+    const RingCfg& cfg = A.cfg;
+    CgShared sh = cg_carve(smem_raw, a.g.batch);
+    Ring rg;
+    ring_init(rg, smem_raw + A.ring_smem_offset, cfg);
+    cg::grid_group grid = cg::this_grid();
+    const DGrid& g = a.g;
+    const int batch = g.batch;
+    const double cells = (double)g.n[0] * g.n[1] * g.n[2] * (A.cm.n > 1 ? A.cm.n : 1);
+    const float coffs = a.prm.matrix_offset;
+    constexpr bool adaptive = ADAPT;
+    int region = 0;
+    ThreadGroups tg;
+    groups_init(tg, cfg, g, a.pf);
+
+    auto sweep = [&](const unsigned char* active, auto&& body) {
+        int cur_b = cfg.split ? 0 : -1; float acc0 = 0.f, acc1 = 0.f;
+        RingUnit u;
+        for (int k = 0; ring_next_unit<DIM>(cfg, g, k, u); ++k) {
+            if (active && !active[u.b]) continue;
+            if (u.b != cur_b) {
+                if (cur_b >= 0) flush_partials(sh, a.partials, region, batch, cur_b, acc0, acc1);
+                cur_b = u.b; acc0 = 0.f; acc1 = 0.f;
+            }
+            body(u, acc0, acc1);
+        }
+        if (cur_b >= 0) flush_partials(sh, a.partials, region, batch, cur_b, acc0, acc1);
+    };
+    const CommDev& cm = A.cm;
+    unsigned long long seq = cm.n > 1 ? *cm.seq : 0ull;
+    bool comm_ok = true;
+    auto barrier_and_reduce = [&](const unsigned char* active) {
+        fence_proxy_async();
+        if (DIST && cm.n > 1 && A.comm_merge) {
+            comm_ok = comm_barrier_allreduce(cm, sh, a.partials, region, batch, cfg.split ? (int)gridDim.x : cfg.units_per_batch, active, ++seq) && comm_ok;
+            region ^= 1;
+            fence_proxy_async();
+            return;
+        }
+        if (cm.n > 1) __threadfence_system();
+        grid.sync();
+        fence_proxy_async();
+        reduce_partials(sh, a.partials, region, batch, cfg.split ? (int)gridDim.x : cfg.units_per_batch, active);
+        region ^= 1;
+        if (cm.n > 1) {
+            comm_ok = comm_allreduce(cm, sh, batch, ++seq) && comm_ok;
+            fence_proxy_async();
+        }
+    };
+    const long long nzsz = (long long)g.n[2] * a.pf.sz;
+    using PH = typename std::conditional<DIST, PeerHalo, NoPeerHalo>::type;
+    auto peer_halo = [&](float* lo_arr, float* hi_arr) {
+        PH ph;
+        if constexpr (DIST) {
+            ph.plo = cm.lower >= 0 ? lo_arr + nzsz : nullptr;
+            ph.phi = cm.upper >= 0 ? hi_arr - nzsz : nullptr;
+        }
+        ph.zf = 0;
+        return ph;
+    };
+
+    for (int b = threadIdx.x; b < batch; b += blockDim.x) { sh.mean[b] = 0.f; sh.offs[b] = 0.f; }
+    __syncthreads();
+
+    if (a.prm.balance_rhs || coffs != 0.f) {
+        sweep(nullptr, [&](const RingUnit& u, float& acc0, float& acc1) {
+            ring_unit_cells<DIM, RR>(cfg, g, a.pf, tg, u, [&](long long off, int nvalid) {
+                for (int j = 0; j < nvalid; ++j) { acc0 += a.rhs[off + j]; acc1 += MASK ? a.acc[off + j] : a.x[off + j]; }
+            });
+        });
+        barrier_and_reduce(nullptr);
+        for (int b = threadIdx.x; b < batch; b += blockDim.x) {
+            if (MASK) { sh.mean[b] = (a.prm.balance_rhs && sh.sum1[b] > 0.0) ? (float)(sh.sum0[b] / sh.sum1[b]) : 0.f; sh.offs[b] = 0.f; }
+            else { sh.mean[b] = a.prm.balance_rhs ? (float)(sh.sum0[b] / cells) : 0.f; sh.offs[b] = coffs * (float)sh.sum1[b]; }
+        }
+        __syncthreads();
+    }
+
+    {
+        const float* hsrc[2] = {a.x, (OP == CgOp::Masked ? a.acc : (OP == CgOp::HelmholtzVarying ? A.op.k : nullptr))};
+        const float* esrc[2] = {a.rhs, nullptr};
+        sweep(nullptr, [&](const RingUnit& u, float& acc0, float& acc1) {
+            REpiResidual0<PH> epi{a.r, sh.mean[u.b], sh.offs[u.b], 0.f, 0.f, peer_halo(cm.lo_r, cm.hi_r), adaptive};
+            if constexpr (OP == CgOp::Poisson) ring_process_unit<GENERIC, DIM, 1, 1, true, OP, RR>(rg, cfg, g, a.pf, tg, hsrc, esrc, 0.f, u, epi);
+            else cg_op_unit<DIM, GENERIC, OP, 1, 1>(rg, A, tg, hsrc, esrc, 0.f, u, epi);
+            acc0 += epi.acc0; acc1 += epi.acc1;
+        });
+    }
+    barrier_and_reduce(nullptr);
+    for (int b = threadIdx.x; b < batch; b += blockDim.x) {
+        const double d0 = sh.sum0[b], d0tol = sh.sum1[b];
+        sh.delta[b] = d0;
+        const float tol = fmaxf(a.prm.rtol * a.prm.rtol * (float)d0tol, a.prm.atol * a.prm.atol);
+        sh.tol_sq[b] = tol; sh.rsq0[b] = (float)d0;
+        const bool conv = (float)d0 <= tol;
+        const bool divg = !isfinite((float)d0);
+        sh.conv[b] = conv; sh.divg[b] = divg; sh.iters[b] = 0;
+        sh.cont[b] = (!conv && !divg && a.prm.max_iter > 0) ? 1 : 0;
+        sh.beta[b] = 0.f; sh.alpha[b] = 0.f; sh.aprev[b] = 0.f;
+    }
+    __syncthreads();
+    if (threadIdx.x == 0) { int any = 0; for (int b = 0; b < batch; ++b) any |= sh.cont[b]; *sh.any_cont = any; }
+    __syncthreads();
+
+    if constexpr (FUSED) {
+        static_assert(DIM == 3 && !GENERIC && !DIST && !ADAPT && OP == CgOp::Poisson, "the one-sweep CG is 3-D, branch-free, single-GPU CG only");
+        float* const D[3] = {a.d0, a.d1, A.d2};
+        float* const tile = rg.stage0 + (size_t)cfg.R * cfg.stage_floats;
+        FusedGroups fg;
+        fused_groups_init(fg, cfg, g, a.pf);
+        if (*sh.any_cont) {
+            const float* hsrc[2] = {a.r, nullptr};
+            const float* esrc[2] = {nullptr, nullptr};
+            sweep(sh.cont, [&](const RingUnit& u, float& acc0, float& acc1) {
+                REpiFusedStart epi{D[0], 0.f, 0.f};
+                ring_process_unit<false, 3, 1, 0, true, OP, RR>(rg, cfg, g, a.pf, tg, hsrc, esrc, 0.f, u, epi);
+                acc0 += epi.acc0; acc1 += epi.acc1;
+            });
+            barrier_and_reduce(sh.cont);
+            for (int b = threadIdx.x; b < batch; b += blockDim.x) {
+                if (!sh.cont[b]) continue;
+                const double dl = sh.delta[b], dq = sh.sum0[b];
+                const float al = (dq != 0.0) ? (float)(dl / dq) : 0.f;
+                const double nxt = dl - 2.0 * al * dq + (double)al * al * sh.sum1[b];
+                sh.alpha[b] = al;
+                sh.beta[b] = (dl != 0.0) ? (float)(nxt / dl) : 0.f;
+                sh.bprev[b] = 0.f;
+            }
+            __syncthreads();
+        }
+        const int upb = cfg.split ? (int)gridDim.x : cfg.units_per_batch;
+        int reg = 1;
+        for (int k = 0; *sh.any_cont; ++k) {
+            FusedPass P;
+            P.d = D[k % 3]; P.dprev = k > 0 ? D[(k + 2) % 3] : nullptr;
+            P.dn = D[(k + 1) % 3]; P.x = (k & 1) ? a.x : nullptr;
+            int cur_b = cfg.split ? 0 : -1;
+            float acc[4] = {0.f, 0.f, 0.f, 0.f};
+            RingUnit u;
+            for (int j = 0; ring_next_unit<3>(cfg, g, j, u); ++j) {
+                if (!sh.cont[u.b]) continue;
+                if (u.b != cur_b) {
+                    if (cur_b >= 0) { flush_partials(sh, a.partials, 2 * reg, batch, cur_b, acc[0], acc[1]);
+                                      flush_partials(sh, a.partials, 2 * reg + 1, batch, cur_b, acc[2], acc[3]); }
+                    cur_b = u.b; acc[0] = acc[1] = acc[2] = acc[3] = 0.f;
+                }
+                P.alpha = sh.alpha[u.b]; P.aprev = sh.aprev[u.b]; P.beta = sh.beta[u.b]; P.bprev = sh.bprev[u.b];
+                ring_fused_unit<RR>(rg, cfg, g, a.pf, fg, P, tile, u, acc);
+            }
+            if (cur_b >= 0) { flush_partials(sh, a.partials, 2 * reg, batch, cur_b, acc[0], acc[1]);
+                              flush_partials(sh, a.partials, 2 * reg + 1, batch, cur_b, acc[2], acc[3]); }
+            fence_proxy_async();
+            grid.sync();
+            fence_proxy_async();
+            reduce_partials(sh, a.partials, 2 * reg, batch, upb, sh.cont);
+            for (int b = threadIdx.x; b < batch; b += blockDim.x) {
+                if (!sh.cont[b]) continue;
+                const double dn = sh.sum1[b], dq = sh.sum0[b];
+                sh.delta[b] = dn;
+                const int it = ++sh.iters[b];
+                const float rsq = fabsf((float)dn);
+                const bool conv = rsq <= sh.tol_sq[b];
+                const bool divg = !isfinite(rsq) || (rsq / sh.rsq0[b] > 1e5f && it >= 8);
+                sh.conv[b] = conv; sh.divg[b] = divg;
+                sh.cont[b] = (!conv && !divg && it < a.prm.max_iter) ? 1 : 0;
+                if (sh.cont[b]) {
+                    sh.aprev[b] = sh.alpha[b];
+                    sh.bprev[b] = sh.beta[b];
+                    sh.alpha[b] = (dq != 0.0) ? (float)(dn / dq) : 0.f;
+                }
+            }
+            __syncthreads();
+            reduce_partials(sh, a.partials, 2 * reg + 1, batch, upb, sh.cont);
+            for (int b = threadIdx.x; b < batch; b += blockDim.x) {
+                if (!sh.cont[b]) continue;
+                const double dn = sh.delta[b], al = sh.alpha[b];
+                const double nxt = dn - 2.0 * al * sh.sum0[b] + al * al * sh.sum1[b];
+                sh.beta[b] = (dn != 0.0) ? (float)(nxt / dn) : 0.f;
+            }
+            __syncthreads();
+            if (threadIdx.x == 0) { int any = 0; for (int b = 0; b < batch; ++b) any |= sh.cont[b]; *sh.any_cont = any; }
+            __syncthreads();
+            reg ^= 1;
+        }
+        region = reg == 1 ? 2 : 0;
+        RingUnit u;
+        for (int k = 0; ring_next_unit<DIM>(cfg, g, k, u); ++k) {
+            const int it = sh.iters[u.b];
+            if (!(it & 1)) continue;
+            const float al = sh.alpha[u.b];
+            const float* dl = D[(it - 1) % 3];
+            ring_unit_cells<DIM, RR>(cfg, g, a.pf, tg, u, [&](long long off, int) {
+                float4 xv = *reinterpret_cast<const float4*>(a.x + off);
+                const float4 dv = *reinterpret_cast<const float4*>(dl + off);
+                xv.x += al * dv.x; xv.y += al * dv.y; xv.z += al * dv.z; xv.w += al * dv.w;
+                *reinterpret_cast<float4*>(a.x + off) = xv;
+            });
+        }
+    }
+
+    float* dold = a.d0; float* dnew = a.d1;
+    float* lo_dnew = cm.lo_d1; float* hi_dnew = cm.hi_d1; float* lo_dold = cm.lo_d0; float* hi_dold = cm.hi_d0;
+    bool x_pending = false;
+    while (!FUSED && *sh.any_cont && comm_ok) {
+        if (cfg.dbg & 1) {} else if constexpr (!ADAPT) {
+            const float* hsrc[3] = {a.r, dold, (OP == CgOp::Masked ? a.acc : (OP == CgOp::HelmholtzVarying ? A.op.k : nullptr))};
+            const float* esrc[2] = {nullptr, nullptr};
+            sweep(sh.cont, [&](const RingUnit& u, float& acc0, float& acc1) {
+                REpiPassA<PH> epi{dnew, 0.f, 0.f, peer_halo(lo_dnew, hi_dnew)};
+                if constexpr (OP == CgOp::Poisson) ring_process_unit<GENERIC, DIM, 2, 0>(rg, cfg, g, a.pf, tg, hsrc, esrc, sh.beta[u.b], u, epi);
+                else cg_op_unit<DIM, GENERIC, OP, 2, 0>(rg, A, tg, hsrc, esrc, sh.beta[u.b], u, epi);
+                acc0 += epi.acc0; acc1 += epi.acc1;
+            });
+        } else if constexpr (OP == CgOp::Poisson) {
+            const float* hsrc[2] = {a.r, dold};
+            const float* esrc[2] = {a.r, nullptr};
+            sweep(sh.cont, [&](const RingUnit& u, float& acc0, float& acc1) {
+                REpiPassAAdapt<PH> epi{dnew, 0.f, 0.f, peer_halo(lo_dnew, hi_dnew)};
+                ring_process_unit<GENERIC, DIM, 2, 1>(rg, cfg, g, a.pf, tg, hsrc, esrc, sh.beta[u.b], u, epi);
+                acc0 += epi.acc0; acc1 += epi.acc1;
+            });
+        } else {
+            const float* hsrc[3] = {a.r, dold, a.acc};
+            const float* esrc[2] = {a.r, nullptr};
+            sweep(sh.cont, [&](const RingUnit& u, float& acc0, float& acc1) {
+                REpiPassAAdapt<PH> epi{dnew, 0.f, 0.f, peer_halo(lo_dnew, hi_dnew)};
+                cg_op_unit<DIM, GENERIC, OP, 2, 1>(rg, A, tg, hsrc, esrc, sh.beta[u.b], u, epi);
+                acc0 += epi.acc0; acc1 += epi.acc1;
+            });
+        }
+        barrier_and_reduce(sh.cont);
+        for (int b = threadIdx.x; b < batch; b += blockDim.x) {
+            if (!sh.cont[b]) continue;
+            sh.aprev[b] = sh.alpha[b];
+            if (adaptive) {
+                const double dq = sh.sum0[b];
+                sh.alpha[b] = (dq != 0.0) ? (float)(sh.sum1[b] / dq) : 0.f;
+                sh.delta[b] = dq;
+                sh.offs[b] = 0.f;
+                continue;
+            }
+            const double S = sh.sum1[b];
+            const double dq = sh.sum0[b] + (double)coffs * S * S;
+            sh.alpha[b] = (dq != 0.0) ? (float)(sh.delta[b] / dq) : 0.f;
+            sh.offs[b] = coffs * (float)S;
+        }
+        __syncthreads();
+        if (cfg.dbg & 2) {} else if (!x_pending) {
+            const float* hsrc[2] = {dnew, (OP == CgOp::Masked ? a.acc : (OP == CgOp::HelmholtzVarying ? A.op.k : nullptr))};
+            const float* esrc[3] = {a.r, nullptr, nullptr};
+            sweep(sh.cont, [&](const RingUnit& u, float& acc0, float& acc1) {
+                REpiPassBr<PH, ADAPT> epi{a.r, sh.alpha[u.b], ADAPT ? 0.f : sh.offs[u.b], 0.f, 0.f, peer_halo(cm.lo_r, cm.hi_r)};
+                if constexpr (OP == CgOp::Poisson) ring_process_unit<GENERIC, DIM, 1, 1>(rg, cfg, g, a.pf, tg, hsrc, esrc, 0.f, u, epi);
+                else cg_op_unit<DIM, GENERIC, OP, 1, 1>(rg, A, tg, hsrc, esrc, 0.f, u, epi);
+                acc0 += epi.acc0; if (ADAPT) acc1 += epi.acc1;
+            });
+        } else {
+            const float* hsrc[2] = {dnew, (OP == CgOp::Masked ? a.acc : (OP == CgOp::HelmholtzVarying ? A.op.k : nullptr))};
+            const float* esrc[3] = {a.x, a.r, dold};
+            sweep(sh.cont, [&](const RingUnit& u, float& acc0, float& acc1) {
+                REpiPassB<PH, ADAPT> epi{a.x, a.r, sh.alpha[u.b], sh.aprev[u.b], ADAPT ? 0.f : sh.offs[u.b], 0.f, 0.f, peer_halo(cm.lo_r, cm.hi_r)};
+                if constexpr (OP == CgOp::Poisson) ring_process_unit<GENERIC, DIM, 1, 3>(rg, cfg, g, a.pf, tg, hsrc, esrc, 0.f, u, epi);
+                else cg_op_unit<DIM, GENERIC, OP, 1, 3>(rg, A, tg, hsrc, esrc, 0.f, u, epi);
+                acc0 += epi.acc0; if (ADAPT) acc1 += epi.acc1;
+            });
+        }
+        x_pending = !x_pending;
+        barrier_and_reduce(sh.cont);
+        for (int b = threadIdx.x; b < batch; b += blockDim.x) {
+            if (!sh.cont[b]) continue;
+            const double dn = sh.sum0[b];
+            const double dprev = sh.delta[b];
+            if (adaptive) sh.beta[b] = (dprev != 0.0) ? -(float)(sh.sum1[b] / dprev) : 0.f;
+            else sh.beta[b] = (dprev != 0.0) ? (float)(dn / dprev) : 0.f;
+            sh.delta[b] = dn;
+            const int it = ++sh.iters[b];
+            const float rsq = fabsf((float)dn);
+            const bool conv = rsq <= sh.tol_sq[b];
+            const bool divg = !isfinite(rsq) || (rsq / sh.rsq0[b] > 1e5f && it >= 8);
+            sh.conv[b] = conv; sh.divg[b] = divg;
+            sh.cont[b] = (!conv && !divg && it < a.prm.max_iter) ? 1 : 0;
+        }
+        __syncthreads();
+        if (threadIdx.x == 0) { int any = 0; for (int b = 0; b < batch; ++b) any |= sh.cont[b]; *sh.any_cont = any; }
+        __syncthreads();
+        float* t = dold; dold = dnew; dnew = t;
+        t = lo_dold; lo_dold = lo_dnew; lo_dnew = t;
+        t = hi_dold; hi_dold = hi_dnew; hi_dnew = t;
+    }
+
+    RingUnit u;
+    for (int k = 0; !FUSED && ring_next_unit<DIM>(cfg, g, k, u); ++k) {
+        if (!(sh.iters[u.b] & 1)) continue;
+        const float al = sh.alpha[u.b];
+        ring_unit_cells<DIM>(cfg, g, a.pf, tg, u, [&](long long off, int nvalid) {
+            if (nvalid == 4) {
+                float4 xv = *reinterpret_cast<const float4*>(a.x + off);
+                const float4 dv = *reinterpret_cast<const float4*>(a.d1 + off);
+                xv.x += al * dv.x; xv.y += al * dv.y; xv.z += al * dv.z; xv.w += al * dv.w;
+                *reinterpret_cast<float4*>(a.x + off) = xv;
+            } else for (int j = 0; j < nvalid; ++j) a.x[off + j] += al * a.d1[off + j];
+        });
+    }
+
+    if (a.prm.project_mean) {
+        sweep(nullptr, [&](const RingUnit& u, float& acc0, float& acc1) {
+            ring_unit_cells<DIM, RR>(cfg, g, a.pf, tg, u, [&](long long off, int nvalid) {
+                for (int j = 0; j < nvalid; ++j) { if (MASK) { acc0 += a.x[off + j] * a.acc[off + j]; acc1 += a.acc[off + j]; } else acc0 += a.x[off + j]; }
+            });
+        });
+        barrier_and_reduce(nullptr);
+        for (int k = 0; ring_next_unit<DIM>(cfg, g, k, u); ++k) {
+            const float m = MASK ? (sh.sum1[u.b] > 0.0 ? (float)(sh.sum0[u.b] / sh.sum1[u.b]) : 0.f) : (float)(sh.sum0[u.b] / cells);
+            ring_unit_cells<DIM, RR>(cfg, g, a.pf, tg, u, [&](long long off, int nvalid) {
+                for (int j = 0; j < nvalid; ++j) a.x[off + j] -= MASK ? m * a.acc[off + j] : m;
+            });
+        }
+    }
+
+    if (cm.n > 1 && blockIdx.x == 0 && threadIdx.x == 0) *cm.seq = seq;
+    if (blockIdx.x == 0) {
+        for (int b = threadIdx.x; b < batch; b += blockDim.x) {
+            PhiCgResult res;
+            res.iterations = sh.iters[b]; res.converged = sh.conv[b]; res.diverged = comm_ok ? sh.divg[b] : -1;
+            res.residual_sq = fabsf((float)sh.delta[b]); res.tol_sq = sh.tol_sq[b]; res.initial_residual_sq = sh.rsq0[b];
+            a.result[b] = res;
+        }
+    }
diff --git a/phiflow_b200/csrc/ring_kernels.cu b/phiflow_b200/csrc/ring_kernels.cu
--- a/phiflow_b200/csrc/ring_kernels.cu
+++ b/phiflow_b200/csrc/ring_kernels.cu
@@ -11,6 +11,19 @@
 #define RING_THREADS (RING_CONSUMERS + 32)
 #define RING_MAX_STAGES 8
 #define RING_G 4
+#define RING_FUSED_THREADS (RING_CONSUMERS + 128)
+#define RING_FUSED_LAUNCH_REGS (65536 / RING_FUSED_THREADS / 8 * 8)
+#define RING_FUSED_CONSUMER_REGS 200
+#define RING_FUSED_PRODUCER_REGS 104
+static_assert(RING_CONSUMERS * (RING_FUSED_CONSUMER_REGS - RING_FUSED_LAUNCH_REGS) <= 128 * (RING_FUSED_LAUNCH_REGS - RING_FUSED_PRODUCER_REGS),
+              "the consumers' setmaxnreg.inc takes no more registers than the producer warpgroup releases");
+
+enum class RingRole { All, Consumers, Producers };
+template <RingRole RR>
+__device__ __forceinline__ bool ring_producer_side(int consumers)
+{ return RR == RingRole::All ? (int)threadIdx.x >= consumers : RR == RingRole::Producers; }
+template <RingRole RR>
+__device__ __forceinline__ bool ring_idle(int consumers) { return RR == RingRole::Producers && (int)threadIdx.x >= consumers + 32; }
 
 struct RingCfg {
     int TY, R, pitch, nx4;
@@ -512,15 +525,16 @@
     rg.pos = c2;
 }
 
-template <bool GENERIC, int DIM, int NH, int NE, bool MARCH = true, CgOp OP = CgOp::Poisson, class Epi>
+template <bool GENERIC, int DIM, int NH, int NE, bool MARCH = true, CgOp OP = CgOp::Poisson, RingRole RR = RingRole::All, class Epi>
 __device__ __forceinline__ void ring_process_unit(Ring& rg, const RingCfg& cfg, const DGrid& g, const DField& pf,
                                                   ThreadGroups& tg,
                                                   const float* const* hsrc, const float* const* esrc, float beta,
                                                   const RingUnit& u, Epi& epi, int kb = 0, const CgOperator* od = nullptr)
 {
     constexpr bool XSLOT = cg_op_xslot(OP);
-    const bool producer = (int)threadIdx.x >= cfg.consumers;
+    const bool producer = ring_producer_side<RR>(cfg.consumers);
     if (producer) {
+        if (ring_idle<RR>(cfg.consumers)) return;
         const int nh = (NH == 2 && beta == 0.f) ? 1 : NH;
         ProdUnit pu;
         prod_unit_setup<DIM, OP == CgOp::HelmholtzVarying>(pu, cfg, g, pf, ((1u << nh) - 1u) | (XSLOT ? (1u << NH) : 0u), NH + (XSLOT ? 1 : 0), NE, hsrc, esrc, u.b, u.y0, kb);
@@ -838,11 +852,11 @@
     return ok;
 }
 
-template <int DIM, class F>
+template <int DIM, RingRole RR = RingRole::All, class F>
 __device__ __forceinline__ void ring_unit_cells(const RingCfg& cfg, const DGrid& g, const DField& pf, const ThreadGroups& tg,
                                                 const RingUnit& u, F&& fn)
 {
-    if ((int)threadIdx.x >= cfg.consumers) return;
+    if (ring_producer_side<RR>(cfg.consumers)) return;
     long long plane_off = (long long)u.b * pf.sb + (long long)u.y0 * pf.sy + (DIM == 3 ? (long long)u.z0 * pf.sz : 0);
     for (int z = u.z0; z < u.z1; ++z, plane_off += pf.sz)
 #pragma unroll
@@ -995,11 +1009,13 @@
     float alpha, aprev, beta, bprev;
 };
 
+template <RingRole RR>
 __device__ __forceinline__ void ring_fused_unit(Ring& rg, const RingCfg& cfg, const DGrid& g, const DField& pf, const FusedGroups& fg,
                                                 const FusedPass& P, float* tile, const RingUnit& u, float (&acc)[4])
 {
     const int nz = u.z1 - u.z0;
-    if ((int)threadIdx.x >= cfg.consumers) {
+    if (ring_producer_side<RR>(cfg.consumers)) {
+        if (ring_idle<RR>(cfg.consumers)) return;
         ProdUnitF pu;
         prod_fused_setup(pu, cfg, g, pf, P.d, P.dprev, u.b, u.y0);
         for (int p = 0; p < nz + 4; ++p)
@@ -1140,343 +1156,30 @@
     }
 };
 
+template <int DIM, bool GENERIC, bool DIST, bool ADAPT, CgOp OP, bool FUSED, RingRole RR>
+__device__ __forceinline__ void cg_ring_role(const CgRingArgs& A)
+{
+#include "cg_ring_body.cuh"
+}
+
+__device__ __forceinline__ void setmaxnreg_dec_producer() { asm volatile("setmaxnreg.dec.sync.aligned.u32 %0;" ::"n"(RING_FUSED_PRODUCER_REGS)); }
+__device__ __forceinline__ void setmaxnreg_inc_consumer() { asm volatile("setmaxnreg.inc.sync.aligned.u32 %0;" ::"n"(RING_FUSED_CONSUMER_REGS)); }
+
 template <int DIM, bool GENERIC, bool DIST, bool ADAPT, CgOp OP = CgOp::Poisson, bool FUSED = false>
-__global__ void __launch_bounds__(RING_THREADS, 1)
+__global__ void __launch_bounds__(FUSED ? RING_FUSED_THREADS : RING_THREADS, 1)
 k_cg_ring(CgRingArgs A)
 {
-    constexpr bool MASK = OP == CgOp::Masked;
-    static_assert((OP != CgOp::Helmholtz && OP != CgOp::HelmholtzVarying) || (!DIST && !ADAPT && !FUSED),
-                  "the Helmholtz operators run on the single-GPU two-sweep CG only");
-    static_assert(!MASK || !ADAPT || (!DIST && !FUSED), "CG-adaptive with obstacles runs on the single-GPU two-sweep CG only");
-    static_assert(!cg_op_xslot(OP) || GENERIC, "the face-minimum stencil runs on the generic consumer");
-    extern __shared__ __align__(128) unsigned char smem_raw[];
-    const CgArgs& a = A.a;
-    const RingCfg& cfg = A.cfg;
-    CgShared sh = cg_carve(smem_raw, a.g.batch);
-    Ring rg;
-    ring_init(rg, smem_raw + A.ring_smem_offset, cfg);
-    cg::grid_group grid = cg::this_grid();
-    const DGrid& g = a.g;
-    const int batch = g.batch;
-    const double cells = (double)g.n[0] * g.n[1] * g.n[2] * (A.cm.n > 1 ? A.cm.n : 1);
-    const float coffs = a.prm.matrix_offset;
-    constexpr bool adaptive = ADAPT;
-    int region = 0;
-    ThreadGroups tg;
-    groups_init(tg, cfg, g, a.pf);
-
-    auto sweep = [&](const unsigned char* active, auto&& body) {
-        int cur_b = cfg.split ? 0 : -1; float acc0 = 0.f, acc1 = 0.f;
-        RingUnit u;
-        for (int k = 0; ring_next_unit<DIM>(cfg, g, k, u); ++k) {
-            if (active && !active[u.b]) continue;
-            if (u.b != cur_b) {
-                if (cur_b >= 0) flush_partials(sh, a.partials, region, batch, cur_b, acc0, acc1);
-                cur_b = u.b; acc0 = 0.f; acc1 = 0.f;
-            }
-            body(u, acc0, acc1);
-        }
-        if (cur_b >= 0) flush_partials(sh, a.partials, region, batch, cur_b, acc0, acc1);
-    };
-    const CommDev& cm = A.cm;
-    unsigned long long seq = cm.n > 1 ? *cm.seq : 0ull;
-    bool comm_ok = true;
-    auto barrier_and_reduce = [&](const unsigned char* active) {
-        fence_proxy_async();
-        if (DIST && cm.n > 1 && A.comm_merge) {
-            comm_ok = comm_barrier_allreduce(cm, sh, a.partials, region, batch, cfg.split ? (int)gridDim.x : cfg.units_per_batch, active, ++seq) && comm_ok;
-            region ^= 1;
-            fence_proxy_async();
-            return;
-        }
-        if (cm.n > 1) __threadfence_system();
-        grid.sync();
-        fence_proxy_async();
-        reduce_partials(sh, a.partials, region, batch, cfg.split ? (int)gridDim.x : cfg.units_per_batch, active);
-        region ^= 1;
-        if (cm.n > 1) {
-            comm_ok = comm_allreduce(cm, sh, batch, ++seq) && comm_ok;
-            fence_proxy_async();
-        }
-    };
-    const long long nzsz = (long long)g.n[2] * a.pf.sz;
-    using PH = typename std::conditional<DIST, PeerHalo, NoPeerHalo>::type;
-    auto peer_halo = [&](float* lo_arr, float* hi_arr) {
-        PH ph;
-        if constexpr (DIST) {
-            ph.plo = cm.lower >= 0 ? lo_arr + nzsz : nullptr;
-            ph.phi = cm.upper >= 0 ? hi_arr - nzsz : nullptr;
-        }
-        ph.zf = 0;
-        return ph;
-    };
-
-    for (int b = threadIdx.x; b < batch; b += blockDim.x) { sh.mean[b] = 0.f; sh.offs[b] = 0.f; }
-    __syncthreads();
-
-    if (a.prm.balance_rhs || coffs != 0.f) {
-        sweep(nullptr, [&](const RingUnit& u, float& acc0, float& acc1) {
-            ring_unit_cells<DIM>(cfg, g, a.pf, tg, u, [&](long long off, int nvalid) {
-                for (int j = 0; j < nvalid; ++j) { acc0 += a.rhs[off + j]; acc1 += MASK ? a.acc[off + j] : a.x[off + j]; }
-            });
-        });
-        barrier_and_reduce(nullptr);
-        for (int b = threadIdx.x; b < batch; b += blockDim.x) {
-            if (MASK) { sh.mean[b] = (a.prm.balance_rhs && sh.sum1[b] > 0.0) ? (float)(sh.sum0[b] / sh.sum1[b]) : 0.f; sh.offs[b] = 0.f; }
-            else { sh.mean[b] = a.prm.balance_rhs ? (float)(sh.sum0[b] / cells) : 0.f; sh.offs[b] = coffs * (float)sh.sum1[b]; }
-        }
-        __syncthreads();
-    }
-
-    {
-        const float* hsrc[2] = {a.x, (OP == CgOp::Masked ? a.acc : (OP == CgOp::HelmholtzVarying ? A.op.k : nullptr))};
-        const float* esrc[2] = {a.rhs, nullptr};
-        sweep(nullptr, [&](const RingUnit& u, float& acc0, float& acc1) {
-            REpiResidual0<PH> epi{a.r, sh.mean[u.b], sh.offs[u.b], 0.f, 0.f, peer_halo(cm.lo_r, cm.hi_r), adaptive};
-            if constexpr (OP == CgOp::Poisson) ring_process_unit<GENERIC, DIM, 1, 1>(rg, cfg, g, a.pf, tg, hsrc, esrc, 0.f, u, epi);
-            else cg_op_unit<DIM, GENERIC, OP, 1, 1>(rg, A, tg, hsrc, esrc, 0.f, u, epi);
-            acc0 += epi.acc0; acc1 += epi.acc1;
-        });
-    }
-    barrier_and_reduce(nullptr);
-    for (int b = threadIdx.x; b < batch; b += blockDim.x) {
-        const double d0 = sh.sum0[b], d0tol = sh.sum1[b];
-        sh.delta[b] = d0;
-        const float tol = fmaxf(a.prm.rtol * a.prm.rtol * (float)d0tol, a.prm.atol * a.prm.atol);
-        sh.tol_sq[b] = tol; sh.rsq0[b] = (float)d0;
-        const bool conv = (float)d0 <= tol;
-        const bool divg = !isfinite((float)d0);
-        sh.conv[b] = conv; sh.divg[b] = divg; sh.iters[b] = 0;
-        sh.cont[b] = (!conv && !divg && a.prm.max_iter > 0) ? 1 : 0;
-        sh.beta[b] = 0.f; sh.alpha[b] = 0.f; sh.aprev[b] = 0.f;
-    }
-    __syncthreads();
-    if (threadIdx.x == 0) { int any = 0; for (int b = 0; b < batch; ++b) any |= sh.cont[b]; *sh.any_cont = any; }
-    __syncthreads();
-
     if constexpr (FUSED) {
-        static_assert(DIM == 3 && !GENERIC && !DIST && !ADAPT && OP == CgOp::Poisson, "the one-sweep CG is 3-D, branch-free, single-GPU CG only");
-        float* const D[3] = {a.d0, a.d1, A.d2};
-        float* const tile = rg.stage0 + (size_t)cfg.R * cfg.stage_floats;
-        FusedGroups fg;
-        fused_groups_init(fg, cfg, g, a.pf);
-        if (*sh.any_cont) {
-            const float* hsrc[2] = {a.r, nullptr};
-            const float* esrc[2] = {nullptr, nullptr};
-            sweep(sh.cont, [&](const RingUnit& u, float& acc0, float& acc1) {
-                REpiFusedStart epi{D[0], 0.f, 0.f};
-                ring_process_unit<false, 3, 1, 0, true>(rg, cfg, g, a.pf, tg, hsrc, esrc, 0.f, u, epi);
-                acc0 += epi.acc0; acc1 += epi.acc1;
-            });
-            barrier_and_reduce(sh.cont);
-            for (int b = threadIdx.x; b < batch; b += blockDim.x) {
-                if (!sh.cont[b]) continue;
-                const double dl = sh.delta[b], dq = sh.sum0[b];
-                const float al = (dq != 0.0) ? (float)(dl / dq) : 0.f;
-                const double nxt = dl - 2.0 * al * dq + (double)al * al * sh.sum1[b];
-                sh.alpha[b] = al;
-                sh.beta[b] = (dl != 0.0) ? (float)(nxt / dl) : 0.f;
-                sh.bprev[b] = 0.f;
-            }
-            __syncthreads();
-        }
-        const int upb = cfg.split ? (int)gridDim.x : cfg.units_per_batch;
-        int reg = 1;
-        for (int k = 0; *sh.any_cont; ++k) {
-            FusedPass P;
-            P.d = D[k % 3]; P.dprev = k > 0 ? D[(k + 2) % 3] : nullptr;
-            P.dn = D[(k + 1) % 3]; P.x = (k & 1) ? a.x : nullptr;
-            int cur_b = cfg.split ? 0 : -1;
-            float acc[4] = {0.f, 0.f, 0.f, 0.f};
-            RingUnit u;
-            for (int j = 0; ring_next_unit<3>(cfg, g, j, u); ++j) {
-                if (!sh.cont[u.b]) continue;
-                if (u.b != cur_b) {
-                    if (cur_b >= 0) { flush_partials(sh, a.partials, 2 * reg, batch, cur_b, acc[0], acc[1]);
-                                      flush_partials(sh, a.partials, 2 * reg + 1, batch, cur_b, acc[2], acc[3]); }
-                    cur_b = u.b; acc[0] = acc[1] = acc[2] = acc[3] = 0.f;
-                }
-                P.alpha = sh.alpha[u.b]; P.aprev = sh.aprev[u.b]; P.beta = sh.beta[u.b]; P.bprev = sh.bprev[u.b];
-                ring_fused_unit(rg, cfg, g, a.pf, fg, P, tile, u, acc);
-            }
-            if (cur_b >= 0) { flush_partials(sh, a.partials, 2 * reg, batch, cur_b, acc[0], acc[1]);
-                              flush_partials(sh, a.partials, 2 * reg + 1, batch, cur_b, acc[2], acc[3]); }
-            fence_proxy_async();
-            grid.sync();
-            fence_proxy_async();
-            reduce_partials(sh, a.partials, 2 * reg, batch, upb, sh.cont);
-            for (int b = threadIdx.x; b < batch; b += blockDim.x) {
-                if (!sh.cont[b]) continue;
-                const double dn = sh.sum1[b], dq = sh.sum0[b];
-                sh.delta[b] = dn;
-                const int it = ++sh.iters[b];
-                const float rsq = fabsf((float)dn);
-                const bool conv = rsq <= sh.tol_sq[b];
-                const bool divg = !isfinite(rsq) || (rsq / sh.rsq0[b] > 1e5f && it >= 8);
-                sh.conv[b] = conv; sh.divg[b] = divg;
-                sh.cont[b] = (!conv && !divg && it < a.prm.max_iter) ? 1 : 0;
-                if (sh.cont[b]) {
-                    sh.aprev[b] = sh.alpha[b];
-                    sh.bprev[b] = sh.beta[b];
-                    sh.alpha[b] = (dq != 0.0) ? (float)(dn / dq) : 0.f;
-                }
-            }
-            __syncthreads();
-            reduce_partials(sh, a.partials, 2 * reg + 1, batch, upb, sh.cont);
-            for (int b = threadIdx.x; b < batch; b += blockDim.x) {
-                if (!sh.cont[b]) continue;
-                const double dn = sh.delta[b], al = sh.alpha[b];
-                const double nxt = dn - 2.0 * al * sh.sum0[b] + al * al * sh.sum1[b];
-                sh.beta[b] = (dn != 0.0) ? (float)(nxt / dn) : 0.f;
-            }
-            __syncthreads();
-            if (threadIdx.x == 0) { int any = 0; for (int b = 0; b < batch; ++b) any |= sh.cont[b]; *sh.any_cont = any; }
-            __syncthreads();
-            reg ^= 1;
-        }
-        region = reg == 1 ? 2 : 0;
-        RingUnit u;
-        for (int k = 0; ring_next_unit<DIM>(cfg, g, k, u); ++k) {
-            const int it = sh.iters[u.b];
-            if (!(it & 1)) continue;
-            const float al = sh.alpha[u.b];
-            const float* dl = D[(it - 1) % 3];
-            ring_unit_cells<DIM>(cfg, g, a.pf, tg, u, [&](long long off, int) {
-                float4 xv = *reinterpret_cast<const float4*>(a.x + off);
-                const float4 dv = *reinterpret_cast<const float4*>(dl + off);
-                xv.x += al * dv.x; xv.y += al * dv.y; xv.z += al * dv.z; xv.w += al * dv.w;
-                *reinterpret_cast<float4*>(a.x + off) = xv;
-            });
-        }
-    }
-
-    float* dold = a.d0; float* dnew = a.d1;
-    float* lo_dnew = cm.lo_d1; float* hi_dnew = cm.hi_d1; float* lo_dold = cm.lo_d0; float* hi_dold = cm.hi_d0;
-    bool x_pending = false;
-    while (!FUSED && *sh.any_cont && comm_ok) {
-        if (cfg.dbg & 1) {} else if constexpr (!ADAPT) {
-            const float* hsrc[3] = {a.r, dold, (OP == CgOp::Masked ? a.acc : (OP == CgOp::HelmholtzVarying ? A.op.k : nullptr))};
-            const float* esrc[2] = {nullptr, nullptr};
-            sweep(sh.cont, [&](const RingUnit& u, float& acc0, float& acc1) {
-                REpiPassA<PH> epi{dnew, 0.f, 0.f, peer_halo(lo_dnew, hi_dnew)};
-                if constexpr (OP == CgOp::Poisson) ring_process_unit<GENERIC, DIM, 2, 0>(rg, cfg, g, a.pf, tg, hsrc, esrc, sh.beta[u.b], u, epi);
-                else cg_op_unit<DIM, GENERIC, OP, 2, 0>(rg, A, tg, hsrc, esrc, sh.beta[u.b], u, epi);
-                acc0 += epi.acc0; acc1 += epi.acc1;
-            });
-        } else if constexpr (OP == CgOp::Poisson) {
-            const float* hsrc[2] = {a.r, dold};
-            const float* esrc[2] = {a.r, nullptr};
-            sweep(sh.cont, [&](const RingUnit& u, float& acc0, float& acc1) {
-                REpiPassAAdapt<PH> epi{dnew, 0.f, 0.f, peer_halo(lo_dnew, hi_dnew)};
-                ring_process_unit<GENERIC, DIM, 2, 1>(rg, cfg, g, a.pf, tg, hsrc, esrc, sh.beta[u.b], u, epi);
-                acc0 += epi.acc0; acc1 += epi.acc1;
-            });
+        if (threadIdx.x >= RING_CONSUMERS) {
+            setmaxnreg_dec_producer();
+            cg_ring_role<DIM, GENERIC, DIST, ADAPT, OP, FUSED, RingRole::Producers>(A);
         } else {
-            const float* hsrc[3] = {a.r, dold, a.acc};
-            const float* esrc[2] = {a.r, nullptr};
-            sweep(sh.cont, [&](const RingUnit& u, float& acc0, float& acc1) {
-                REpiPassAAdapt<PH> epi{dnew, 0.f, 0.f, peer_halo(lo_dnew, hi_dnew)};
-                cg_op_unit<DIM, GENERIC, OP, 2, 1>(rg, A, tg, hsrc, esrc, sh.beta[u.b], u, epi);
-                acc0 += epi.acc0; acc1 += epi.acc1;
-            });
-        }
-        barrier_and_reduce(sh.cont);
-        for (int b = threadIdx.x; b < batch; b += blockDim.x) {
-            if (!sh.cont[b]) continue;
-            sh.aprev[b] = sh.alpha[b];
-            if (adaptive) {
-                const double dq = sh.sum0[b];
-                sh.alpha[b] = (dq != 0.0) ? (float)(sh.sum1[b] / dq) : 0.f;
-                sh.delta[b] = dq;
-                sh.offs[b] = 0.f;
-                continue;
-            }
-            const double S = sh.sum1[b];
-            const double dq = sh.sum0[b] + (double)coffs * S * S;
-            sh.alpha[b] = (dq != 0.0) ? (float)(sh.delta[b] / dq) : 0.f;
-            sh.offs[b] = coffs * (float)S;
-        }
-        __syncthreads();
-        if (cfg.dbg & 2) {} else if (!x_pending) {
-            const float* hsrc[2] = {dnew, (OP == CgOp::Masked ? a.acc : (OP == CgOp::HelmholtzVarying ? A.op.k : nullptr))};
-            const float* esrc[3] = {a.r, nullptr, nullptr};
-            sweep(sh.cont, [&](const RingUnit& u, float& acc0, float& acc1) {
-                REpiPassBr<PH, ADAPT> epi{a.r, sh.alpha[u.b], ADAPT ? 0.f : sh.offs[u.b], 0.f, 0.f, peer_halo(cm.lo_r, cm.hi_r)};
-                if constexpr (OP == CgOp::Poisson) ring_process_unit<GENERIC, DIM, 1, 1>(rg, cfg, g, a.pf, tg, hsrc, esrc, 0.f, u, epi);
-                else cg_op_unit<DIM, GENERIC, OP, 1, 1>(rg, A, tg, hsrc, esrc, 0.f, u, epi);
-                acc0 += epi.acc0; if (ADAPT) acc1 += epi.acc1;
-            });
-        } else {
-            const float* hsrc[2] = {dnew, (OP == CgOp::Masked ? a.acc : (OP == CgOp::HelmholtzVarying ? A.op.k : nullptr))};
-            const float* esrc[3] = {a.x, a.r, dold};
-            sweep(sh.cont, [&](const RingUnit& u, float& acc0, float& acc1) {
-                REpiPassB<PH, ADAPT> epi{a.x, a.r, sh.alpha[u.b], sh.aprev[u.b], ADAPT ? 0.f : sh.offs[u.b], 0.f, 0.f, peer_halo(cm.lo_r, cm.hi_r)};
-                if constexpr (OP == CgOp::Poisson) ring_process_unit<GENERIC, DIM, 1, 3>(rg, cfg, g, a.pf, tg, hsrc, esrc, 0.f, u, epi);
-                else cg_op_unit<DIM, GENERIC, OP, 1, 3>(rg, A, tg, hsrc, esrc, 0.f, u, epi);
-                acc0 += epi.acc0; if (ADAPT) acc1 += epi.acc1;
-            });
-        }
-        x_pending = !x_pending;
-        barrier_and_reduce(sh.cont);
-        for (int b = threadIdx.x; b < batch; b += blockDim.x) {
-            if (!sh.cont[b]) continue;
-            const double dn = sh.sum0[b];
-            const double dprev = sh.delta[b];
-            if (adaptive) sh.beta[b] = (dprev != 0.0) ? -(float)(sh.sum1[b] / dprev) : 0.f;
-            else sh.beta[b] = (dprev != 0.0) ? (float)(dn / dprev) : 0.f;
-            sh.delta[b] = dn;
-            const int it = ++sh.iters[b];
-            const float rsq = fabsf((float)dn);
-            const bool conv = rsq <= sh.tol_sq[b];
-            const bool divg = !isfinite(rsq) || (rsq / sh.rsq0[b] > 1e5f && it >= 8);
-            sh.conv[b] = conv; sh.divg[b] = divg;
-            sh.cont[b] = (!conv && !divg && it < a.prm.max_iter) ? 1 : 0;
-        }
-        __syncthreads();
-        if (threadIdx.x == 0) { int any = 0; for (int b = 0; b < batch; ++b) any |= sh.cont[b]; *sh.any_cont = any; }
-        __syncthreads();
-        float* t = dold; dold = dnew; dnew = t;
-        t = lo_dold; lo_dold = lo_dnew; lo_dnew = t;
-        t = hi_dold; hi_dold = hi_dnew; hi_dnew = t;
-    }
-
-    RingUnit u;
-    for (int k = 0; !FUSED && ring_next_unit<DIM>(cfg, g, k, u); ++k) {
-        if (!(sh.iters[u.b] & 1)) continue;
-        const float al = sh.alpha[u.b];
-        ring_unit_cells<DIM>(cfg, g, a.pf, tg, u, [&](long long off, int nvalid) {
-            if (nvalid == 4) {
-                float4 xv = *reinterpret_cast<const float4*>(a.x + off);
-                const float4 dv = *reinterpret_cast<const float4*>(a.d1 + off);
-                xv.x += al * dv.x; xv.y += al * dv.y; xv.z += al * dv.z; xv.w += al * dv.w;
-                *reinterpret_cast<float4*>(a.x + off) = xv;
-            } else for (int j = 0; j < nvalid; ++j) a.x[off + j] += al * a.d1[off + j];
-        });
-    }
-
-    if (a.prm.project_mean) {
-        sweep(nullptr, [&](const RingUnit& u, float& acc0, float& acc1) {
-            ring_unit_cells<DIM>(cfg, g, a.pf, tg, u, [&](long long off, int nvalid) {
-                for (int j = 0; j < nvalid; ++j) { if (MASK) { acc0 += a.x[off + j] * a.acc[off + j]; acc1 += a.acc[off + j]; } else acc0 += a.x[off + j]; }
-            });
-        });
-        barrier_and_reduce(nullptr);
-        for (int k = 0; ring_next_unit<DIM>(cfg, g, k, u); ++k) {
-            const float m = MASK ? (sh.sum1[u.b] > 0.0 ? (float)(sh.sum0[u.b] / sh.sum1[u.b]) : 0.f) : (float)(sh.sum0[u.b] / cells);
-            ring_unit_cells<DIM>(cfg, g, a.pf, tg, u, [&](long long off, int nvalid) {
-                for (int j = 0; j < nvalid; ++j) a.x[off + j] -= MASK ? m * a.acc[off + j] : m;
-            });
-        }
-    }
-
-    if (cm.n > 1 && blockIdx.x == 0 && threadIdx.x == 0) *cm.seq = seq;
-    if (blockIdx.x == 0) {
-        for (int b = threadIdx.x; b < batch; b += blockDim.x) {
-            PhiCgResult res;
-            res.iterations = sh.iters[b]; res.converged = sh.conv[b]; res.diverged = comm_ok ? sh.divg[b] : -1;
-            res.residual_sq = fabsf((float)sh.delta[b]); res.tol_sq = sh.tol_sq[b]; res.initial_residual_sq = sh.rsq0[b];
-            a.result[b] = res;
-        }
+            setmaxnreg_inc_consumer();
+            cg_ring_role<DIM, GENERIC, DIST, ADAPT, OP, FUSED, RingRole::Consumers>(A);
+        }
+    } else {
+        constexpr RingRole RR = RingRole::All;
+#include "cg_ring_body.cuh"
     }
 }
 
@@ -1656,7 +1359,7 @@
             }
         }
     }
-    const int threads = RING_THREADS;
+    const int threads = fused ? RING_FUSED_THREADS : RING_THREADS;
     const size_t smem = (size_t)cgs + 128 + (size_t)A.cfg.R * A.cfg.stage_floats * 4 + tile_bytes;
     const void* fn = (const void*)cg_ring_kernel(op, g.dim, generic, dist, adapt, fused);
     if (!fn) return -100;
```

New measurement: 1.993 (median of 6 runs). About the same (+0.7%).
